# Samsonboadi/Image_to_pointCloud

Measured on NVIDIA B200. Metric: depth_to_point_cloud_throughput, higher is better.
Workload: dtype f64

## Files before the change

image_to_pointcloud_b200/csrc/d2pc_device.cuh:

```cuda
#ifndef D2PC_DEVICE_CUH_
#define D2PC_DEVICE_CUH_

#include <cuda_runtime.h>
#include <stdint.h>

#include "d2pc_math.h"

namespace d2pc {

constexpr int kSampleSize = 8192;
constexpr int kSample2Size = 4096;
constexpr int kSortCap = 16384;
constexpr int kSelBits = 12;
constexpr int kScanThreads = 256;
constexpr int kScanPerThread = 32;
constexpr int kScanTile = kScanThreads * kScanPerThread;
constexpr int kSelThreads = 1024;
constexpr int kSelectThreads = 512;
constexpr int kEmitThreads = 256;
constexpr int kEmitPerThread = 4;
constexpr int kEmitTile = kEmitThreads * kEmitPerThread;
constexpr int kFbTargets = 4;
constexpr uint32_t kCandDivisor = 16;

struct Geom {
  int32_t H, W, C, h, w, step;
  int32_t nu, nv;
  uint32_t P;
  uint32_t N;
  uint32_t D;
  int32_t native;
  double scale_x, scale_y;
};

inline Geom make_geom(const D2pcConfig &c) {
  Geom g;
  g.H = c.img_h; g.W = c.img_w; g.C = c.img_c; g.h = c.dep_h; g.w = c.dep_w; g.step = c.step;
  g.nu = (c.img_w + c.step - 1) / c.step;
  g.nv = (c.img_h + c.step - 1) / c.step;
  g.P = (uint32_t)c.img_h * (uint32_t)c.img_w;
  g.N = (uint32_t)g.nu * (uint32_t)g.nv;
  g.D = (uint32_t)c.dep_h * (uint32_t)c.dep_w;
  g.native = (c.dep_h == c.img_h && c.dep_w == c.img_w) ? 1 : 0;
  g.scale_x = (double)c.dep_w / (double)c.img_w;
  g.scale_y = (double)c.dep_h / (double)c.img_h;
  return g;
}

struct __align__(256) FrameState {
  uint32_t brL[2], brU[2];
  uint32_t sample_ok;
  uint32_t below[2];
  uint32_t above1;
  uint32_t eqL[2];
  uint32_t inside[2];
  uint32_t eqU[2];
  uint32_t n_nonfinite, n_nan;
  alignas(8) uint32_t nqueue[2];
  uint32_t min_key, max_key;
  uint32_t sel_key[4];
  uint32_t sel_fail;
  uint32_t sel_done;
  uint32_t fb_prefix[kFbTargets];
  uint32_t fb_rank[kFbTargets];
  uint32_t fb_active;
  uint32_t fb_any_nan;
  int32_t mask_mode;
  float mask_lo, mask_hi;
  uint32_t emit_count;
  uint32_t bounds_min[3], bounds_max[3];
  alignas(128) NormParams norm;
  int32_t status;
};
static_assert(sizeof(NormParams) + 4 <= 128, "norm + status must share one 128-byte line");
constexpr int kStatusWord = (int)(sizeof(NormParams) / 4);

constexpr uint32_t kSelBins = 4096, kSelListCap = 1024;
struct __align__(256) SelShared {
  uint32_t counts[2][8];
  uint32_t scan_done;
  uint32_t a_done[2], c_done[2];
  uint32_t bin_ready[2];
  uint32_t bin[2][2], base[2][2], need[2][2], want[2][2], shared_bin[2], key[2][2];
  uint32_t mcount[2][2], mmin[2][2], mmax[2][2];
  uint32_t pad_[7];
  uint32_t members[2][2][kSelListCap];
  uint32_t hist[2][kSelBins];
};

struct __align__(8) TapEntry {
  int32_t i0c;
  float t;
};

constexpr int kSchedQueues = 32;
constexpr size_t kSchedBytes = 128 * (kSchedQueues + 1);

struct WsLayout {
  size_t state_off, cand_off, tile_off, fbhist_off, tap_off, sched_off, sel_off, resized_off, total;
  uint32_t cand_cap;
  uint32_t emit_tiles;
};

inline size_t align_up(size_t x, size_t a) { return (x + a - 1) / a * a; }

inline WsLayout make_layout(const D2pcConfig &c) {
  Geom g = make_geom(c);
  WsLayout L;
  uint32_t cap = g.P / kCandDivisor + 1;
  uint32_t small = g.P < (uint32_t)kSortCap ? g.P : (uint32_t)kSortCap;
  if (cap < small) cap = small;
  cap = (cap + 3u) & ~3u;
  L.cand_cap = cap;
  L.emit_tiles = (g.N + kEmitTile - 1) / kEmitTile;
  size_t off = 0;
  L.state_off = off;  off = align_up(off + sizeof(FrameState) * (size_t)c.batch, 256);
  L.cand_off = off;   off = align_up(off + (size_t)c.batch * 2 * cap * sizeof(uint32_t), 256);
  L.tile_off = off;   off = align_up(off + (size_t)c.batch * L.emit_tiles * sizeof(unsigned long long), 256);
  L.fbhist_off = off; off = align_up(off + (size_t)c.batch * kFbTargets * 256 * sizeof(uint32_t), 256);
  L.tap_off = off;    off = align_up(off + ((size_t)c.img_w + (size_t)c.img_h) * sizeof(TapEntry), 256);
  L.sched_off = off;  off = align_up(off + kSchedBytes + (size_t)c.batch * 64, 256);
  L.sel_off = off;    off = align_up(off + (size_t)c.batch * sizeof(SelShared), 256);
  L.resized_off = off;
  if (!g.native) off = align_up(off + (size_t)c.batch * g.P * sizeof(float), 256);
  L.total = off;
  return L;
}

struct KParams {
  Geom g;
  int32_t batch;
  const float *depth;
  FrameState *state;
  uint32_t *cand;
  unsigned long long *tile_state;
  uint32_t *fb_hist;
  const TapEntry *xtab, *ytab;
  SelShared *sel;
  uint32_t *sched;
  float *resized;
  uint32_t cand_cap, emit_tiles;
  int32_t force_fallback;
  int32_t hints;
};

constexpr int kHintScanKeep = 1;
constexpr int kHintEmitDepthFirst = 2;
constexpr int kHintStreamFirst = 4;
constexpr int kHintResizedKeep = 8;
constexpr int kHintPipeline = 15;

inline KParams make_kparams(const D2pcConfig &c, const float *d_depth, void *ws) {
  KParams k;
  WsLayout L = make_layout(c);
  char *base = (char *)ws;
  k.g = make_geom(c);
  k.batch = c.batch;
  k.depth = d_depth;
  k.state = (FrameState *)(base + L.state_off);
  k.cand = (uint32_t *)(base + L.cand_off);
  k.tile_state = (unsigned long long *)(base + L.tile_off);
  k.fb_hist = (uint32_t *)(base + L.fbhist_off);
  k.xtab = (const TapEntry *)(base + L.tap_off);
  k.ytab = k.xtab + c.img_w;
  k.sched = (uint32_t *)(base + L.sched_off);
  k.sel = (SelShared *)(base + L.sel_off);
  k.resized = k.g.native ? nullptr : (float *)(base + L.resized_off);
  k.cand_cap = L.cand_cap;
  k.emit_tiles = L.emit_tiles;
  k.force_fallback = c.force_fallback;
  k.hints = 0;
  return k;
}

inline KParams per_pixel_view(const KParams &kp) {
  KParams v = kp;
  if (!kp.g.native) {
    v.depth = kp.resized;
    v.g.D = kp.g.P;
    v.g.h = kp.g.H;
    v.g.w = kp.g.W;
    v.g.native = 1;
  }
  return v;
}

inline KParams slice_kparams(const KParams &kp, int b0, int nb, int ring_slot) {
  KParams s = kp;
  s.batch = nb;
  s.depth = kp.depth + (size_t)b0 * kp.g.D;
  s.state = kp.state + b0;
  s.cand = kp.cand + (size_t)b0 * 2 * kp.cand_cap;
  s.tile_state = kp.tile_state + (size_t)b0 * kp.emit_tiles;
  s.fb_hist = kp.fb_hist + (size_t)b0 * kFbTargets * 256;
  s.sel = kp.sel + b0;
  if (kp.resized) s.resized = kp.resized + (size_t)(ring_slot >= 0 ? ring_slot : b0) * kp.g.P;
  return s;
}

struct EmitArgs {
  const uint8_t *bgr;
  float *xyz, *rgb;
  uint32_t *count;
  PixelConsts pc;
  int32_t use_z, drop_nf, want_bounds;
  float z_min, z_max;
  uint32_t frame0;
};

int validate_config(const D2pcConfig *cfg);
int check_workspace(const D2pcConfig *cfg, const void *ws, size_t ws_bytes);
int stats_prepare();
int taps_launch(const KParams &kp, cudaStream_t st);
constexpr int kStatsSample = 1, kStatsScan = 2, kStatsSelect = 4, kStatsScanSelect = kStatsScan | kStatsSelect;
int stats_launch(KParams kp, cudaStream_t st, int phases);
int status_launch(const KParams &kp, int32_t *d_status, int32_t *d_any, cudaStream_t st);
EmitArgs make_emit_args(const D2pcConfig &cfg, const uint8_t *d_bgr, float *d_xyz, float *d_rgb, uint32_t *d_count);
EmitArgs slice_emit_args(const EmitArgs &ea, const Geom &g, int b0);
int emit_init_launch(const KParams &kp, cudaStream_t st);
int bounds_export_launch(const KParams &kp, float *d_bounds, cudaStream_t st);
int emit_validate(const D2pcConfig *cfg, const float *d_depth, const uint8_t *d_bgr, void *d_workspace,
                  size_t workspace_bytes, float *d_xyz, float *d_rgb, uint32_t *d_count, float *d_bounds);
int emit_launch(const D2pcConfig &cfg, const KParams &kp, const EmitArgs &ea, float *d_bounds, cudaStream_t st,
                int32_t smooth_k, const double *h_kernel, void *d_scratch);
int record_cuda_error(cudaError_t e);

#define D2PC_CHECK_LAUNCH()                                  \
  do {                                                       \
    cudaError_t e__ = cudaGetLastError();                    \
    if (e__ != cudaSuccess) return record_cuda_error(e__);   \
  } while (0)

#if defined(__CUDACC__)
__device__ __forceinline__ float4 ldg_stream_f4(const float *p) {
  float4 r;
  asm volatile("ld.global.nc.L1::no_allocate.v4.f32 {%0,%1,%2,%3}, [%4];"
               : "=f"(r.x), "=f"(r.y), "=f"(r.z), "=f"(r.w) : "l"(p));
  return r;
}
__device__ __forceinline__ uint64_t l2_policy(bool first, bool last) {
  uint64_t pf, pl, pn;
  asm("createpolicy.fractional.L2::evict_first.b64 %0, 1.0;" : "=l"(pf));
  asm("createpolicy.fractional.L2::evict_last.b64 %0, 1.0;" : "=l"(pl));
  asm("createpolicy.fractional.L2::evict_normal.b64 %0, 1.0;" : "=l"(pn));
  return first ? pf : (last ? pl : pn);
}
__device__ __forceinline__ float4 ldg_f4_pol(const float *p, uint64_t pol) {
  float4 r;
  asm volatile("ld.global.nc.L1::no_allocate.L2::cache_hint.v4.f32 {%0,%1,%2,%3}, [%4], %5;"
               : "=f"(r.x), "=f"(r.y), "=f"(r.z), "=f"(r.w) : "l"(p), "l"(pol));
  return r;
}
__device__ __forceinline__ uint32_t ldg_u32_pol(const void *p, uint64_t pol) {
  uint32_t r;
  asm volatile("ld.global.nc.L1::no_allocate.L2::cache_hint.u32 %0, [%1], %2;" : "=r"(r) : "l"(p), "l"(pol));
  return r;
}
__device__ __forceinline__ void stg_f4_pol(float *p, float4 v, uint64_t pol) {
  asm volatile("st.global.L2::cache_hint.v4.f32 [%0], {%1,%2,%3,%4}, %5;"
               :: "l"(p), "f"(v.x), "f"(v.y), "f"(v.z), "f"(v.w), "l"(pol) : "memory");
}
__device__ __forceinline__ void bulk_store_pol(void *gdst, uint32_t smem_addr, uint32_t bytes, uint64_t pol) {
  asm volatile("cp.async.bulk.global.shared::cta.bulk_group.L2::cache_hint [%0], [%1], %2, %3;"
               :: "l"(gdst), "r"(smem_addr), "r"(bytes), "l"(pol) : "memory");
}
__device__ __forceinline__ uint32_t ldg_stream_u32(const void *p) {
  uint32_t r;
  asm volatile("ld.global.nc.L1::no_allocate.u32 %0, [%1];" : "=r"(r) : "l"(p));
  return r;
}
__device__ __forceinline__ void stg_f1_pol(float *p, float v, uint64_t pol) {
  asm volatile("st.global.L2::cache_hint.f32 [%0], %1, %2;" :: "l"(p), "f"(v), "l"(pol) : "memory");
}
__device__ __forceinline__ void stg_stream_f4(float *p, float4 v) {
  asm volatile("st.global.cs.v4.f32 [%0], {%1,%2,%3,%4};"
               :: "l"(p), "f"(v.x), "f"(v.y), "f"(v.z), "f"(v.w) : "memory");
}
__device__ __forceinline__ void stg_stream_f1(float *p, float v) {
  asm volatile("st.global.cs.f32 [%0], %1;" :: "l"(p), "f"(v) : "memory");
}

__device__ __forceinline__ uint32_t warp_sum(uint32_t v) {
#pragma unroll
  for (int o = 16; o > 0; o >>= 1) v += __shfl_xor_sync(0xffffffffu, v, o);
  return v;
}
__device__ __forceinline__ uint32_t warp_min(uint32_t v) {
#pragma unroll
  for (int o = 16; o > 0; o >>= 1) v = min(v, __shfl_xor_sync(0xffffffffu, v, o));
  return v;
}
__device__ __forceinline__ uint32_t warp_max(uint32_t v) {
#pragma unroll
  for (int o = 16; o > 0; o >>= 1) v = max(v, __shfl_xor_sync(0xffffffffu, v, o));
  return v;
}

__device__ __forceinline__ void block_bitonic_sort(uint32_t *s, uint32_t n) {
  const uint32_t half = n >> 1;
  for (uint32_t k = 2; k <= n; k <<= 1) {
    for (uint32_t j = k >> 1; j > 0; j >>= 1) {
      for (uint32_t i = threadIdx.x; i < half; i += blockDim.x) {
        uint32_t a = ((i & ~(j - 1)) << 1) | (i & (j - 1));
        uint32_t b = a | j;
        uint32_t x = s[a], y = s[b];
        bool up = (a & k) == 0;
        if ((x > y) == up) { s[a] = y; s[b] = x; }
      }
      __syncthreads();
    }
  }
}

template <int T, int NBLOG, typename ForEach>
__device__ __forceinline__ bool block_hist_select(ForEach for_each, uint32_t lo0, uint32_t hi0,
                                                  const uint32_t (&rank)[T], uint32_t (&out)[T],
                                                  uint32_t *s_hist, uint32_t *s_res) {
  constexpr uint32_t NB = 1u << NBLOG;
  const int tid = threadIdx.x, nthr = blockDim.x;
  const int lane = tid & 31, warp = tid >> 5, nwarp = nthr >> 5;
  uint32_t lo[T], span[T], base[T];
  bool done[T];
#pragma unroll
  for (int t = 0; t < T; ++t) { lo[t] = lo0; span[t] = hi0 - lo0; base[t] = 0; done[t] = false; out[t] = 0; }
  bool shared_range = true, ok = true;
  uint32_t *s_warp = s_res + 2 * T;
  for (int level = 0; level < 6; ++level) {
    bool all_done = true;
#pragma unroll
    for (int t = 0; t < T; ++t) all_done = all_done && done[t];
    if (all_done) break;
    int shift[T];
#pragma unroll
    for (int t = 0; t < T; ++t) {
      const int bits = span[t] ? 32 - __clz(span[t]) : 0;
      shift[t] = bits > NBLOG ? bits - NBLOG : 0;
    }
    const int nh = shared_range ? 1 : T;
    for (uint32_t i = tid; i < (uint32_t)nh * NB; i += nthr) s_hist[i] = 0u;
    if (tid < 2 * T) s_res[tid] = 0xFFFFFFFFu;
    __syncthreads();
    if (shared_range) {
      for_each([&](uint32_t key) {
        const uint32_t d = key - lo[0];
        if (d <= span[0]) atomicAdd(&s_hist[d >> shift[0]], 1u);
      });
    } else {
      for_each([&](uint32_t key) {
#pragma unroll
        for (int t = 0; t < T; ++t) {
          const uint32_t d = key - lo[t];
          if (!done[t] && d <= span[t]) atomicAdd(&s_hist[t * NB + (d >> shift[t])], 1u);
        }
      });
    }
    __syncthreads();
    for (int h = 0; h < nh; ++h) {
      if (!shared_range && done[h]) continue;
      const uint32_t *hist = s_hist + (size_t)h * NB;
      constexpr int PER = 4;
      uint32_t carry = 0;
      for (uint32_t chunk = 0; chunk < NB; chunk += (uint32_t)nthr * PER) {
        const uint32_t b0 = chunk + (uint32_t)tid * PER;
        uint32_t c[PER], sum = 0;
#pragma unroll
        for (int i = 0; i < PER; ++i) { c[i] = (b0 + i < NB) ? hist[b0 + i] : 0u; sum += c[i]; }
        uint32_t incl = sum;
#pragma unroll
        for (int d = 1; d < 32; d <<= 1) {
          uint32_t y = __shfl_up_sync(0xffffffffu, incl, d);
          if (lane >= d) incl += y;
        }
        if (lane == 31) s_warp[warp] = incl;
        __syncthreads();
        uint32_t woff = 0, total = 0;
        for (int w = 0; w < nwarp; ++w) { const uint32_t x = s_warp[w]; if (w < warp) woff += x; total += x; }
        uint32_t pref = carry + woff + incl - sum;
#pragma unroll
        for (int i = 0; i < PER; ++i) {
#pragma unroll
          for (int t = 0; t < T; ++t) {
            const bool mine = shared_range ? !done[t] : (t == h);
            const uint32_t r = rank[t] - base[t];
            if (mine && c[i] && pref <= r && r < pref + c[i]) { s_res[2 * t] = b0 + i; s_res[2 * t + 1] = pref; }
          }
          pref += c[i];
        }
        carry += total;
        __syncthreads();
      }
    }
    __syncthreads();
#pragma unroll
    for (int t = 0; t < T; ++t) {
      if (done[t]) continue;
      const uint32_t bin = s_res[2 * t], pref = s_res[2 * t + 1];
      if (bin == 0xFFFFFFFFu) { ok = false; done[t] = true; continue; }
      base[t] += pref;
      lo[t] += bin << shift[t];
      span[t] = shift[t] ? ((1u << shift[t]) - 1u) : 0u;
      if (shift[t] == 0) { done[t] = true; out[t] = lo[t]; }
    }
    shared_range = false;
    __syncthreads();
  }
  return ok;
}

constexpr int kFastBinsLog = 12;
constexpr uint32_t kFastBins = 1u << kFastBinsLog;
constexpr uint32_t kFastListCap = 1024;

__device__ __forceinline__ int fast_shift(uint32_t span) {
  const int bits = span ? 32 - __clz(span) : 0;
  return bits > kFastBinsLog ? bits - kFastBinsLog : 0;
}

template <int T, bool GLOBAL = false>
__device__ __forceinline__ void block_locate(const uint32_t *s_hist, const uint32_t (&rank)[T], const bool (&want)[T],
                                             uint32_t (&bin)[T], uint32_t (&base)[T], uint32_t *s_warp,
                                             uint32_t *s_res) {
  const int tid = threadIdx.x, lane = tid & 31, warp = tid >> 5, nwarp = blockDim.x >> 5;
  const int per = (int)(kFastBins / blockDim.x);
  if (tid < 2 * T) s_res[tid] = 0xFFFFFFFFu;
  const uint32_t b0 = (uint32_t)tid * (uint32_t)per;
  uint32_t sum = 0;
  for (int i = 0; i < per; i += 4) {
    const uint4 c = GLOBAL ? __ldcg(reinterpret_cast<const uint4 *>(s_hist + b0 + i))
                           : *reinterpret_cast<const uint4 *>(s_hist + b0 + i);
    sum += c.x + c.y + c.z + c.w;
  }
  uint32_t incl = sum;
#pragma unroll
  for (int d = 1; d < 32; d <<= 1) {
    const uint32_t y = __shfl_up_sync(0xffffffffu, incl, d);
    if (lane >= d) incl += y;
  }
  if (lane == 31) s_warp[warp] = incl;
  __syncthreads();
  if (warp == 0) {
    const uint32_t x = lane < nwarp ? s_warp[lane] : 0u;
    uint32_t in2 = x;
#pragma unroll
    for (int d = 1; d < 32; d <<= 1) {
      const uint32_t y = __shfl_up_sync(0xffffffffu, in2, d);
      if (lane >= d) in2 += y;
    }
    __syncwarp();
    s_warp[lane] = in2 - x;
  }
  __syncthreads();
  uint32_t pref = s_warp[warp] + incl - sum;
  bool mine = false;
#pragma unroll
  for (int t = 0; t < T; ++t) mine = mine || (want[t] && sum && pref <= rank[t] && rank[t] < pref + sum);
  if (mine) {
    for (int i = 0; i < per; ++i) {
      const uint32_t c = GLOBAL ? __ldcg(s_hist + b0 + i) : s_hist[b0 + i];
#pragma unroll
      for (int t = 0; t < T; ++t)
        if (want[t] && c && pref <= rank[t] && rank[t] < pref + c) { s_res[2 * t] = b0 + i; s_res[2 * t + 1] = pref; }
      pref += c;
    }
  }
  __syncthreads();
#pragma unroll
  for (int t = 0; t < T; ++t) { bin[t] = s_res[2 * t]; base[t] = s_res[2 * t + 1]; }
}

__device__ __forceinline__ void block_pick(const uint32_t *list, uint32_t n, uint32_t r, uint32_t *s_out) {
  for (uint32_t i = threadIdx.x; i < n; i += blockDim.x) {
    const uint32_t k = list[i];
    uint32_t smaller = 0, equal = 0;
    for (uint32_t j = 0; j < n; ++j) {
      const uint32_t x = list[j];
      smaller += x < k ? 1u : 0u;
      equal += x == k ? 1u : 0u;
    }
    if (smaller <= r && r < smaller + equal) *s_out = k;
  }
}

__device__ __forceinline__ uint32_t hash_u32(uint32_t x) {
  x ^= x >> 16; x *= 0x7feb352du; x ^= x >> 15; x *= 0x846ca68bu; x ^= x >> 16;
  return x;
}

__device__ __forceinline__ float bilinear_taps(const float *src, int32_t src_w, TapEntry tx, TapEntry ty) {
  const int32_t x0 = tx.i0c & 0x7FFFFFFF, y0 = ty.i0c & 0x7FFFFFFF;
  const bool cx = tx.i0c < 0, cy = ty.i0c < 0;
  const float *row0 = src + (size_t)y0 * src_w;
  const float a0 = __ldg(row0 + x0);
  float r0 = a0;
  if (!cx) r0 = fmaf(__ldg(row0 + x0 + 1) - a0, tx.t, a0);
  if (cy) return (cx && is_inf_f32(r0)) ? nan_f32() : r0;
  const float *row1 = row0 + src_w;
  const float a1 = __ldg(row1 + x0);
  float r1 = a1;
  if (!cx) r1 = fmaf(__ldg(row1 + x0 + 1) - a1, tx.t, a1);
  return fmaf(r1 - r0, ty.t, r0);
}

template <bool NATIVE>
__device__ __forceinline__ float depth_at(const float *frame, const KParams &kp, uint32_t p) {
  if (NATIVE) {
    return __ldg(frame + p);
  } else {
    const uint32_t v = p / (uint32_t)kp.g.W;
    const uint32_t u = p - v * (uint32_t)kp.g.W;
    return bilinear_taps(frame, kp.g.w, kp.xtab[u], kp.ytab[v]);
  }
}
#endif

}
#endif
```

image_to_pointcloud_b200/csrc/d2pc_path.cu:

```cuda
#include <stdlib.h>
#include <string.h>

#include <vector>

#include "d2pc_emit_dev.cuh"
#include "d2pc_stats_dev.cuh"

using namespace d2pc;

namespace d2pc {

__global__ void sched_reset_kernel(KParams kp) {
  if (threadIdx.x <= kSchedQueues) kp.sched[32 * threadIdx.x] = 0u;
}
int sched_reset_launch(const KParams &kp, cudaStream_t st) {
  sched_reset_kernel<<<1, 64, 0, st>>>(kp);
  D2PC_CHECK_LAUNCH();
  return D2PC_OK;
}

struct SchedParams {
  int32_t F, D;
  uint32_t ns, ne, R;
  uint32_t K;
  uint32_t skip;
  uint32_t nq;
  uint32_t group_items, total_items;
  int32_t vec_ok;
};

constexpr int kPathMinBlocks = 6;
__device__ __forceinline__ unsigned long long global_ns() {
  unsigned long long t;
  asm volatile("mov.u64 %0, %globaltimer;" : "=l"(t));
  return t;
}
__device__ __forceinline__ unsigned long long *trace_slot(const KParams &kp, uint32_t f, int k) {
  return reinterpret_cast<unsigned long long *>(reinterpret_cast<unsigned char *>(kp.sched) + kSchedBytes) + (size_t)f * 8 + k;
}

constexpr int kPathScanPT = 16;

template <bool BOUNDS, bool TRACE>
__global__ void __launch_bounds__(kEmitThreads, kPathMinBlocks) path_kernel(KParams kp, EmitArgs ea, FastArgs fa,
                                                                           SchedParams sp) {
  extern __shared__ __align__(16) unsigned char s_dyn[];
  __shared__ EmitSmall s_emit;
  __shared__ SelPartSmall s_sel;
  __shared__ uint32_t s_go;
  __shared__ NormParams s_norm;
  const int tid = threadIdx.x;
  uint32_t *abort_flag = kp.sched + 32u * kSchedQueues;
  const uint32_t item = blockIdx.x;
  const uint32_t g = item / sp.group_items, i = item - g * sp.group_items;
  if (i < 2u * sp.K) {
    if (g < 1u || g > (uint32_t)sp.F || (sp.skip & 1u)) return;
    const int f = (int)g - 1;
    const uint32_t br = i / sp.K, k = i - br * sp.K;
    if (tid == 0) s_go = spin_until(&kp.sel[f].scan_done, abort_flag, [&](uint32_t v) { return v >= sp.ns; }) ? 1u : 0u;
    __syncthreads();
    if (!s_go) return;
    if (TRACE && tid == 0 && k == 0u) *trace_slot(kp, f, 2 + 2 * (int)br) = global_ns();
    select_part(kp, f, (int)br, k, sp.K, reinterpret_cast<float *>(s_dyn), kSliceCap, s_sel,
                [&](const uint32_t *p, auto pred) { return spin_until(p, abort_flag, pred); });
    if (TRACE) {
      __syncthreads();
      if (tid == 0) atomicMax(trace_slot(kp, f, 3 + 2 * (int)br), global_ns());
    }
    return;
  }
  const uint32_t j = i - 2u * sp.K, q = j / (sp.R + 1u), r = j - q * (sp.R + 1u);
  if (r == 0u) {
    if (g >= (uint32_t)sp.F || (sp.skip & 2u)) return;
    if (TRACE && tid == 0) atomicMin(trace_slot(kp, g, 0), global_ns());
    scan_tile<kPathScanPT>(kp, (int)g, q, sp.vec_ok, *reinterpret_cast<ScanTileSmemT<kPathScanPT> *>(s_dyn));
    __syncthreads();
    if (tid == 0) {
      __threadfence();
      atomicAdd(&kp.sel[g].scan_done, 1u);
      if (TRACE) atomicMax(trace_slot(kp, g, 1), global_ns());
    }
    return;
  }
  const uint32_t e = q * sp.R + (r - 1u);
  if (g < (uint32_t)sp.D || e >= sp.ne || (sp.skip & 4u)) return;
  const uint32_t f = g - (uint32_t)sp.D;
  if (f >= (uint32_t)sp.F) return;
  if (TRACE && tid == 0) atomicMin(trace_slot(kp, f, 6), global_ns());
  auto norm_fn = [&]() -> const NormParams * {
    const uint32_t *line = reinterpret_cast<const uint32_t *>(&kp.state[f].norm);
    uint32_t go = 0u;
    for (int attempt = 0; attempt < 2 && go == 0u; ++attempt) {
      if (tid < 32) {
        const uint32_t w = ld_relaxed_u32(line + tid);
        const uint32_t st = __shfl_sync(0xffffffffu, w, kStatusWord);
        if (st == (uint32_t)D2PC_FRAME_READY && tid < kStatusWord) reinterpret_cast<uint32_t *>(&s_norm)[tid] = w;
        if (tid == 0) s_go = st == (uint32_t)D2PC_FRAME_READY ? 1u : (st == (uint32_t)D2PC_FRAME_PENDING ? 0u : 3u);
      }
      __syncthreads();
      go = s_go;
      if (go == 0u) {
        __syncthreads();
        if (tid == 0) s_go = spin_until(line + kStatusWord, abort_flag, [&](uint32_t x) { return x != (uint32_t)D2PC_FRAME_PENDING; }) ? 0u : 2u;
        __syncthreads();
        go = s_go;
        __syncthreads();
      }
    }
    return go == 1u ? &s_norm : nullptr;
  };
  emit_fast_tile<1, false, BOUNDS>(kp, ea, fa, f, e, reinterpret_cast<float *>(s_dyn), s_emit, norm_fn);
  if (TRACE) {
    __syncthreads();
    if (tid == 0) atomicMax(trace_slot(kp, f, 7), global_ns());
  }
}

}

constexpr int kMaxAux = 8, kMaxEmit = 4;

struct D2pcPath {
  int device;
  cudaStream_t s_cap;
  cudaStream_t s_aux[kMaxAux];
  cudaStream_t s_emit[kMaxEmit];
  std::vector<cudaEvent_t> events;
  cudaGraphExec_t exec;
  std::vector<unsigned char> key;
};

namespace {

struct PathArgs {
  D2pcConfig cfg;
  const float *d_depth;
  const uint8_t *d_bgr;
  void *d_workspace;
  size_t workspace_bytes;
  float *d_xyz, *d_rgb;
  uint32_t *d_count;
  float *d_bounds;
  int32_t *d_status, *d_any_fallback;
  int32_t sub_batch, lookahead, flags;
};

int ensure_events(D2pcPath *p, size_t n) {
  while (p->events.size() < n) {
    cudaEvent_t e;
    cudaError_t err = cudaEventCreateWithFlags(&e, cudaEventDisableTiming);
    if (err != cudaSuccess) return record_cuda_error(err);
    p->events.push_back(e);
  }
  return D2PC_OK;
}

#define PATH_CUDA(x)                                         \
  do {                                                       \
    cudaError_t e__ = (x);                                   \
    if (e__ != cudaSuccess) return record_cuda_error(e__);   \
  } while (0)

int path_kernel_supported(const D2pcConfig &cfg, const KParams &kp, const EmitArgs &ea) {
  const bool mask = cfg.use_z_range || cfg.drop_nonfinite;
  return kp.g.native && cfg.step == 1 && !mask && cfg.img_c == 3 && (cfg.img_w % 4) == 0 &&
         (((uintptr_t)kp.depth & 15u) == 0u) && (((uintptr_t)ea.bgr & 3u) == 0u) && (kp.g.N & 3u) == 0u &&
         ((unsigned long long)kp.g.N * (unsigned long long)kp.g.nu < (1ull << 40)) && kp.g.P > (uint32_t)kSortCap;
}

size_t path_kernel_smem() {
  size_t m = sizeof(ScanTileSmemT<kPathScanPT>);
  if (kEmitStageBytes > m) m = kEmitStageBytes;
  return m;
}

static int env_int(const char *name, int dflt, int lo, int hi);

int path_ordered(const PathArgs &a, cudaStream_t st) {
  const D2pcConfig &cfg = a.cfg;
  KParams kp = make_kparams(cfg, a.d_depth, a.d_workspace);
  kp.hints = (a.flags & D2PC_PATH_NO_L2_HINTS) ? 0 : (kHintScanKeep | kHintEmitDepthFirst | kHintStreamFirst);
  if (const char *h = getenv("D2PC_HINTS")) kp.hints = atoi(h);
  const EmitArgs ea = make_emit_args(cfg, a.d_bgr, a.d_xyz, a.d_rgb, a.d_count);
  int rc;
  const int skip = env_int("D2PC_PATH_SKIP", 0, 0, 15);
  if (skip) {
    if ((rc = sched_reset_launch(kp, st)) != D2PC_OK) return rc;
  } else if ((rc = stats_launch(kp, st, kStatsSample)) != D2PC_OK) return rc;
  if (cfg.want_bounds) {
    if ((rc = emit_init_launch(kp, st)) != D2PC_OK) return rc;
  }
  FastArgs fa;
  fa.tiles_per_frame = kp.emit_tiles;
  fa.total_tiles = kp.emit_tiles * (uint32_t)cfg.batch;
  fa.batch = (uint32_t)cfg.batch;
  fa.magic_w = ((1ull << 40) + (unsigned long long)kp.g.nu - 1ull) / (unsigned long long)kp.g.nu;
  fa.pc_simple = consts_simple(ea.pc) ? 1 : 0;
  SchedParams sp;
  sp.F = cfg.batch;
  sp.D = env_int("D2PC_PATH_D", a.lookahead > 0 ? a.lookahead : 3, 2, 64);
  sp.ns = (kp.g.P + kPathScanPT * kScanThreads - 1) / (kPathScanPT * kScanThreads);
  sp.ne = kp.emit_tiles;
  sp.R = (sp.ne + sp.ns - 1) / sp.ns;
  {
    const uint32_t k = (kp.cand_cap + kSliceCap - 1u) / kSliceCap;
    sp.K = (uint32_t)env_int("D2PC_PATH_K", (int)(k < 8u ? 8u : (k > 64u ? 64u : k)), 1, 64);
  }
  sp.skip = (uint32_t)skip;
  sp.nq = (uint32_t)env_int("D2PC_PATH_NQ", 16, 1, kSchedQueues);
  sp.group_items = 2u * sp.K + sp.ns * (sp.R + 1u);
  const unsigned long long total = (unsigned long long)(sp.F + sp.D) * sp.group_items;
  if (total >= 0xFFFF0000ull) return D2PC_ERR_UNSUPPORTED;
  sp.total_items = (uint32_t)total;
  sp.vec_ok = ((kp.g.P & 3u) == 0u) && (((uintptr_t)kp.depth & 15u) == 0u);
  const size_t smem = path_kernel_smem();
  const bool trace = env_int("D2PC_PATH_TRACE", 0, 0, 1) != 0;
  void (*kern)(KParams, EmitArgs, FastArgs, SchedParams) =
      cfg.want_bounds ? (trace ? path_kernel<true, true> : path_kernel<true, false>)
                      : (trace ? path_kernel<false, true> : path_kernel<false, false>);
  PATH_CUDA(cudaFuncSetAttribute(kern, cudaFuncAttributeMaxDynamicSharedMemorySize, (int)smem));
  kern<<<sp.total_items, kEmitThreads, smem, st>>>(kp, ea, fa, sp);
  D2PC_CHECK_LAUNCH();
  if (cfg.want_bounds) {
    if ((rc = bounds_export_launch(kp, a.d_bounds, st)) != D2PC_OK) return rc;
  }
  if (a.d_status || a.d_any_fallback) {
    if ((rc = status_launch(kp, a.d_status, a.d_any_fallback, st)) != D2PC_OK) return rc;
  }
  return D2PC_OK;
}

static int env_int(const char *name, int dflt, int lo, int hi) {
  const char *v = getenv(name);
  int x = v ? atoi(v) : dflt;
  return x < lo ? lo : (x > hi ? hi : x);
}

int path_body(D2pcPath *p, const PathArgs &a, cudaStream_t s_main) {
  const D2pcConfig &cfg = a.cfg;
  KParams kp = make_kparams(cfg, a.d_depth, a.d_workspace);
  const bool generic = !kp.g.native && resize_is_generic(kp.g.h, kp.g.w);
  const int B = cfg.batch, S = generic ? B : a.sub_batch;
  const int n_sub = (B + S - 1) / S;
  const bool overlap = !(a.flags & D2PC_PATH_NO_OVERLAP) && n_sub > 1;
  const int window = (a.lookahead > 0 ? a.lookahead : 1) + 1;
  const int n_aux = overlap ? env_int("D2PC_PATH_AUX", window < kMaxAux ? window : kMaxAux, 1, kMaxAux) : 1;
  const int n_emit = overlap ? env_int("D2PC_PATH_EMIT", 2, 1, kMaxEmit) : 1;
  const bool sample_first = n_sub > 1 && env_int("D2PC_PATH_SAMPLE_FIRST", 1, 0, 1) != 0;
  const bool ring = kp.resized != nullptr && n_sub > 1;
  kp.hints = (a.flags & D2PC_PATH_NO_L2_HINTS) ? 0 : (n_sub > 1 ? kHintPipeline : (kHintEmitDepthFirst | kHintStreamFirst));
  if (ring) kp.hints &= ~kHintEmitDepthFirst;
  if (const char *h = getenv("D2PC_HINTS")) kp.hints = atoi(h);
  const EmitArgs ea = make_emit_args(cfg, a.d_bgr, a.d_xyz, a.d_rgb, a.d_count);
  int rc;
  if ((rc = ensure_events(p, 1 + 3 * (size_t)n_sub)) != D2PC_OK) return rc;
  cudaEvent_t ev_fork = p->events[0];
  cudaEvent_t *ev_stats = &p->events[1], *ev_emit = &p->events[1 + n_sub], *ev_scan = &p->events[1 + 2 * n_sub];
  const bool stagger = overlap && n_aux > 1 && env_int("D2PC_PATH_STAGGER", 0, 0, 1) != 0;
  if ((rc = taps_launch(kp, s_main)) != D2PC_OK) return rc;
  if (sample_first) {
    if ((rc = stats_launch(kp, s_main, kStatsSample)) != D2PC_OK) return rc;
  }
  if (overlap) {
    PATH_CUDA(cudaEventRecord(ev_fork, s_main));
    for (int i = 0; i < n_aux; ++i) PATH_CUDA(cudaStreamWaitEvent(p->s_aux[i], ev_fork, 0));
    if (n_emit > 1)
      for (int i = 0; i < n_emit; ++i) PATH_CUDA(cudaStreamWaitEvent(p->s_emit[i], ev_fork, 0));
  }
  for (int k = 0; k < n_sub; ++k) {
    const int b0 = k * S, nb = (b0 + S <= B) ? S : B - b0;
    const KParams ks = slice_kparams(kp, b0, nb, ring ? (k % window) * S : -1);
    cudaStream_t s_stats = overlap ? p->s_aux[k % n_aux] : s_main;
    cudaStream_t s_em = (overlap && n_emit > 1) ? p->s_emit[k % n_emit] : s_main;
    if (overlap && k >= window) PATH_CUDA(cudaStreamWaitEvent(s_stats, ev_emit[k - window], 0));
    if (stagger) {
      if (!sample_first && (rc = stats_launch(ks, s_stats, kStatsSample)) != D2PC_OK) return rc;
      if (k > 0) PATH_CUDA(cudaStreamWaitEvent(s_stats, ev_scan[k - 1], 0));
      if ((rc = stats_launch(ks, s_stats, kStatsScan)) != D2PC_OK) return rc;
      PATH_CUDA(cudaEventRecord(ev_scan[k], s_stats));
      if ((rc = stats_launch(ks, s_stats, kStatsSelect)) != D2PC_OK) return rc;
    } else if ((rc = stats_launch(ks, s_stats, sample_first ? kStatsScanSelect : (kStatsSample | kStatsScanSelect))) != D2PC_OK)
      return rc;
    if (overlap) {
      PATH_CUDA(cudaEventRecord(ev_stats[k], s_stats));
      PATH_CUDA(cudaStreamWaitEvent(s_em, ev_stats[k], 0));
    }
    if ((rc = emit_launch(cfg, ks, slice_emit_args(ea, kp.g, b0), a.d_bounds ? a.d_bounds + 6 * (size_t)b0 : nullptr,
                          s_em, 0, nullptr, nullptr)) != D2PC_OK)
      return rc;
    if (overlap) PATH_CUDA(cudaEventRecord(ev_emit[k], s_em));
  }
  if (overlap && n_emit > 1) {
    for (int k = n_sub - 1; k >= 0 && k >= n_sub - n_emit; --k) PATH_CUDA(cudaStreamWaitEvent(s_main, ev_emit[k], 0));
  }
  if (a.d_status || a.d_any_fallback) {
    if ((rc = status_launch(kp, a.d_status, a.d_any_fallback, s_main)) != D2PC_OK) return rc;
  }
  return D2PC_OK;
}

}

extern "C" int d2pc_path_create(D2pcPath **path) {
  if (!path) return D2PC_ERR_INVALID_ARGUMENT;
  *path = nullptr;
  D2pcPath *p = new D2pcPath();
  p->exec = nullptr;
  p->s_cap = nullptr;
  for (int i = 0; i < kMaxAux; ++i) p->s_aux[i] = nullptr;
  for (int i = 0; i < kMaxEmit; ++i) p->s_emit[i] = nullptr;
  cudaError_t e = cudaGetDevice(&p->device);
  int lo = 0, hi = 0;
  if (e == cudaSuccess) e = cudaDeviceGetStreamPriorityRange(&lo, &hi);
  if (e == cudaSuccess) e = cudaStreamCreateWithPriority(&p->s_cap, cudaStreamNonBlocking, lo);
  for (int i = 0; i < kMaxAux && e == cudaSuccess; ++i)
    e = cudaStreamCreateWithPriority(&p->s_aux[i], cudaStreamNonBlocking, getenv("D2PC_PATH_NOPRIO") ? lo : hi);
  for (int i = 0; i < kMaxEmit && e == cudaSuccess; ++i)
    e = cudaStreamCreateWithPriority(&p->s_emit[i], cudaStreamNonBlocking, lo);
  if (e != cudaSuccess) {
    d2pc_path_destroy(p);
    return record_cuda_error(e);
  }
  int rc = stats_prepare();
  if (rc) { d2pc_path_destroy(p); return rc; }
  *path = p;
  return D2PC_OK;
}

extern "C" void d2pc_path_destroy(D2pcPath *p) {
  if (!p) return;
  if (p->exec) cudaGraphExecDestroy(p->exec);
  for (cudaEvent_t e : p->events) cudaEventDestroy(e);
  if (p->s_cap) cudaStreamDestroy(p->s_cap);
  for (int i = 0; i < kMaxAux; ++i)
    if (p->s_aux[i]) cudaStreamDestroy(p->s_aux[i]);
  for (int i = 0; i < kMaxEmit; ++i)
    if (p->s_emit[i]) cudaStreamDestroy(p->s_emit[i]);
  delete p;
}

extern "C" int d2pc_path_enqueue(D2pcPath *p, const D2pcConfig *cfg, const float *d_depth, const uint8_t *d_bgr,
                                 void *d_workspace, size_t workspace_bytes, float *d_xyz, float *d_rgb,
                                 uint32_t *d_count, float *d_bounds, int32_t *d_status, int32_t *d_any_fallback,
                                 int32_t sub_batch, int32_t lookahead, int32_t flags, void *stream) {
  if (!p) return D2PC_ERR_INVALID_ARGUMENT;
  int rc = check_workspace(cfg, d_workspace, workspace_bytes);
  if (rc) return rc;
  rc = emit_validate(cfg, d_depth, d_bgr, d_workspace, workspace_bytes, d_xyz, d_rgb, d_count, d_bounds);
  if (rc) return rc;
  int dev = -1;
  PATH_CUDA(cudaGetDevice(&dev));
  if (dev != p->device) return D2PC_ERR_INVALID_ARGUMENT;
  if (sub_batch <= 0 || sub_batch > cfg->batch) sub_batch = cfg->batch;
  if (lookahead < 0) lookahead = 0;
  PathArgs a;
  memset(&a, 0, sizeof(a));
  a.cfg = *cfg;
  a.d_depth = d_depth; a.d_bgr = d_bgr; a.d_workspace = d_workspace; a.workspace_bytes = workspace_bytes;
  a.d_xyz = d_xyz; a.d_rgb = d_rgb; a.d_count = d_count; a.d_bounds = d_bounds;
  a.d_status = d_status; a.d_any_fallback = d_any_fallback;
  a.sub_batch = sub_batch; a.lookahead = lookahead; a.flags = flags;
  cudaStream_t st = (cudaStream_t)stream;
  {
    const KParams kp0 = make_kparams(a.cfg, a.d_depth, a.d_workspace);
    const EmitArgs ea0 = make_emit_args(a.cfg, a.d_bgr, a.d_xyz, a.d_rgb, a.d_count);
    if ((flags & D2PC_PATH_ORDERED) && path_kernel_supported(a.cfg, kp0, ea0)) return path_ordered(a, st);
  }
  if (!(flags & D2PC_PATH_GRAPH)) return path_body(p, a, st);

  const unsigned char *kb = reinterpret_cast<const unsigned char *>(&a);
  if (!p->exec || p->key.size() != sizeof(a) || memcmp(p->key.data(), kb, sizeof(a)) != 0) {
    if (p->exec) { cudaGraphExecDestroy(p->exec); p->exec = nullptr; }
    p->key.clear();
    cudaGraph_t graph = nullptr;
    PATH_CUDA(cudaStreamBeginCapture(p->s_cap, cudaStreamCaptureModeThreadLocal));
    rc = path_body(p, a, p->s_cap);
    cudaError_t e = cudaStreamEndCapture(p->s_cap, &graph);
    if (rc != D2PC_OK) { if (graph) cudaGraphDestroy(graph); return rc; }
    if (e != cudaSuccess) return record_cuda_error(e);
    e = cudaGraphInstantiate(&p->exec, graph, 0);
    cudaGraphDestroy(graph);
    if (e != cudaSuccess) { p->exec = nullptr; return record_cuda_error(e); }
    p->key.assign(kb, kb + sizeof(a));
  }
  PATH_CUDA(cudaGraphLaunch(p->exec, st));
  return D2PC_OK;
}

extern "C" int d2pc_path_trace_offset(const D2pcConfig *cfg, size_t *offset) {
  int rc = validate_config(cfg);
  if (rc) return rc;
  if (!offset) return D2PC_ERR_INVALID_ARGUMENT;
  *offset = make_layout(*cfg).sched_off + kSchedBytes;
  return D2PC_OK;
}
```

image_to_pointcloud_b200/csrc/d2pc_stats.cu:

```cuda
#include <stdlib.h>

#include "d2pc_stats_dev.cuh"

namespace d2pc {

__device__ __forceinline__ int32_t bracket_margin(double q, int S) {
  double sd = sqrt((double)S * q * (1.0 - q));
  return (int32_t)ceil(6.0 * sd) + 4;
}

__global__ void taps_kernel(KParams kp) {
  TapEntry *xt = const_cast<TapEntry *>(kp.xtab), *yt = const_cast<TapEntry *>(kp.ytab);
  const int i = blockIdx.x * blockDim.x + threadIdx.x;
  if (i < kp.g.W) {
    AxisTap a = axis_tap(i, kp.g.scale_x, kp.g.w);
    xt[i].i0c = a.i0 | (a.clamped ? (int32_t)0x80000000 : 0);
    xt[i].t = a.t;
  } else if (i < kp.g.W + kp.g.H) {
    AxisTap a = axis_tap(i - kp.g.W, kp.g.scale_y, kp.g.h);
    yt[i - kp.g.W].i0c = a.i0 | (a.clamped ? (int32_t)0x80000000 : 0);
    yt[i - kp.g.W].t = a.t;
  }
}

__global__ void __launch_bounds__(256) resize_generic_kernel(KParams kp) {
  const uint32_t b = blockIdx.y;
  const float *src = kp.depth + (size_t)b * kp.g.D;
  float *dst = kp.resized + (size_t)b * kp.g.P;
  for (uint32_t p = blockIdx.x * blockDim.x + threadIdx.x; p < kp.g.P; p += gridDim.x * blockDim.x) {
    const uint32_t v = p / (uint32_t)kp.g.W, u = p - v * (uint32_t)kp.g.W;
    dst[p] = generic_sample(src, kp.g.w, generic_tap((int32_t)u, kp.g.scale_x, kp.g.w, 1),
                            generic_tap((int32_t)v, kp.g.scale_y, kp.g.h, 0));
  }
}

template <bool NATIVE>
__global__ void __launch_bounds__(kSelThreads, 1) sample_kernel(KParams kp) {
  extern __shared__ uint32_t s_hist[];
  __shared__ uint32_t s_bad, s_min, s_max;
  __shared__ uint32_t s_res[2 * 4 + 40];
  __shared__ uint32_t s_warp[33], s_cnt[4], s_lmin[4], s_lmax[4], s_out[4];
  const int b = blockIdx.x;
  FrameState *fs = kp.state + b;
  const float *frame = kp.depth + (size_t)b * kp.g.D;
  const uint32_t n = kp.g.P;
  const int tid = threadIdx.x;
  if (tid == 0) {
    s_bad = 0; s_min = 0xFFFFFFFFu; s_max = 0u;
    for (int i = 0; i < 2; ++i) {
      fs->below[i] = 0; fs->eqL[i] = 0; fs->inside[i] = 0; fs->eqU[i] = 0;
    }
    fs->above1 = 0;
    fs->n_nonfinite = 0; fs->n_nan = 0; fs->nqueue[0] = 0; fs->nqueue[1] = 0;
    fs->min_key = 0xFFFFFFFFu; fs->max_key = 0u;
    for (int i = 0; i < 4; ++i) fs->sel_key[i] = 0;
    fs->sel_fail = 0; fs->sel_done = 0;
    if (b == 0)
      for (int i = 0; i <= kSchedQueues; ++i) kp.sched[32 * i] = 0u;
    {
      unsigned long long *tr = reinterpret_cast<unsigned long long *>(reinterpret_cast<unsigned char *>(kp.sched) + kSchedBytes) + (size_t)b * 8;
      for (int i = 0; i < 8; ++i) tr[i] = (i == 0 || i == 6) ? ~0ull : 0ull;
    }
    fs->status = D2PC_FRAME_PENDING;
    fs->fb_active = 0; fs->fb_any_nan = 0;
    fs->norm.has_nonfinite = 0;
    fs->norm.median = 0.0f;
    fs->norm.simple = 0;
  }
  {
    uint32_t *z = reinterpret_cast<uint32_t *>(kp.sel + b);
    for (uint32_t i = tid; i < sizeof(SelShared) / 4; i += kSelThreads) z[i] = 0u;
  }
  if (n <= (uint32_t)kSortCap) {
    if (tid == 0) {
      fs->brL[0] = fs->brL[1] = 0u;
      fs->brU[0] = fs->brU[1] = 0xFFFFFFFFu;
      fs->sample_ok = 1;
    }
    return;
  }
  constexpr int E = kSampleSize / kSelThreads;
  const uint32_t S = kSampleSize;
  uint32_t k[E];
  bool bad = false;
#pragma unroll
  for (int e = 0; e < E; ++e) {
    const uint32_t j = (uint32_t)e * kSelThreads + (uint32_t)tid;
    uint32_t start = (uint32_t)(((unsigned long long)j * n) / S);
    uint32_t end = (uint32_t)(((unsigned long long)(j + 1) * n) / S);
    uint32_t idx = start + hash_u32(j * 0x9E3779B9u + (uint32_t)b * 0x85EBCA6Bu + 12345u) % (end - start);
    float v;
    if (NATIVE) {
      asm volatile("ld.global.nc.L2::64B.f32 %0, [%1];" : "=f"(v) : "l"(frame + idx));
    } else {
      v = depth_at<NATIVE>(frame, kp, idx);
    }
    k[e] = 0xFFFFFFFFu;
    if (is_finite_f32(v)) k[e] = float_to_key(v); else bad = true;
  }
  __syncthreads();
  if (bad) atomicOr(&s_bad, 1u);
  {
    uint32_t mn = 0xFFFFFFFFu, mx = 0u;
#pragma unroll
    for (int e = 0; e < E; ++e) { mn = min(mn, k[e]); mx = max(mx, k[e]); }
    mn = warp_min(mn); mx = warp_max(mx);
    if ((tid & 31) == 0) { atomicMin(&s_min, mn); atomicMax(&s_max, mx); }
  }
  __syncthreads();
  uint32_t rank[4], out[4];
  bool open_lo[2], open_hi[2];
#pragma unroll
  for (int br = 0; br < 2; ++br) {
    const double q = br ? D2PC_Q98 : D2PC_Q02;
    RankPair rp = percentile_ranks(n, q);
    long long i_lo = (long long)(((unsigned long long)rp.lo * S) / n);
    long long i_hi = (long long)(((unsigned long long)rp.hi * S) / n) + 1;
    int32_t m = bracket_margin(q, (int)S);
    long long iL = i_lo - m, iU = i_hi + m;
    open_lo[br] = iL < 0;
    open_hi[br] = iU >= (long long)S;
    rank[2 * br + 0] = open_lo[br] ? 0u : (uint32_t)iL;
    rank[2 * br + 1] = open_hi[br] ? S - 1 : (uint32_t)iU;
  }
  {
    uint32_t *s_list = s_hist + kFastBins;
    const uint32_t lo0 = s_min, span = s_max - s_min;
    const int shift = fast_shift(span);
    for (uint32_t i = tid; i < kFastBins; i += kSelThreads) s_hist[i] = 0u;
    if (tid < 4) { s_cnt[tid] = 0u; s_lmin[tid] = 0xFFFFFFFFu; s_lmax[tid] = 0u; s_out[tid] = 0u; }
    __syncthreads();
#pragma unroll
    for (int e = 0; e < E; ++e) atomicAdd(&s_hist[(k[e] - lo0) >> shift], 1u);
    __syncthreads();
    uint32_t bin[4], base[4];
    const bool want[4] = {true, true, true, true};
    block_locate<4>(s_hist, rank, want, bin, base, s_warp, s_res);
    bool slow = false;
#pragma unroll
    for (int t = 0; t < 4; ++t) slow = slow || bin[t] == 0xFFFFFFFFu;
    if (!slow && shift == 0) {
#pragma unroll
      for (int t = 0; t < 4; ++t) out[t] = lo0 + bin[t];
    } else if (!slow) {
      int owner[4];
#pragma unroll
      for (int t = 0; t < 4; ++t) {
        owner[t] = t;
#pragma unroll
        for (int u = t - 1; u >= 0; --u)
          if (bin[u] == bin[t]) owner[t] = u;
      }
#pragma unroll
      for (int e = 0; e < E; ++e) {
        const uint32_t bk = (k[e] - lo0) >> shift;
#pragma unroll
        for (int t = 0; t < 4; ++t)
          if (owner[t] == t && bk == bin[t]) {
            const uint32_t idx = atomicAdd(&s_cnt[t], 1u);
            if (idx < kFastListCap) s_list[t * kFastListCap + idx] = k[e];
            atomicMin(&s_lmin[t], k[e]);
            atomicMax(&s_lmax[t], k[e]);
          }
      }
      __syncthreads();
#pragma unroll
      for (int t = 0; t < 4; ++t)
        if (owner[t] == t && s_cnt[t] > kFastListCap && s_lmin[t] != s_lmax[t]) slow = true;
      if (!slow) {
#pragma unroll
        for (int t = 0; t < 4; ++t) {
          const int o = owner[t];
          if (s_lmin[o] == s_lmax[o]) { if (tid == 0) s_out[t] = s_lmin[o]; }
          else block_pick(s_list + o * kFastListCap, s_cnt[o], rank[t] - base[t], &s_out[t]);
        }
        __syncthreads();
#pragma unroll
        for (int t = 0; t < 4; ++t) out[t] = s_out[t];
      }
    }
    if (slow) {
      __syncthreads();
      block_hist_select<4, kSelBits>([&](auto f) {
#pragma unroll
        for (int e = 0; e < E; ++e) f(k[e]);
      }, s_min, s_max, rank, out, s_hist, s_res);
    }
  }
  if (tid < 2) {
    fs->brL[tid] = open_lo[tid] ? 0u : out[2 * tid + 0];
    fs->brU[tid] = open_hi[tid] ? 0xFFFFFFFFu : out[2 * tid + 1];
  }
  if (tid == 0) fs->sample_ok = s_bad ? 0u : 1u;
}

template <int QD>
struct ScanSharedT {
  float pqueue[QD][kScanThreads];
  ScanFlushSmem flush;
};
using ScanShared = ScanSharedT<kScanPerThread>;

constexpr int kRzCols = 128, kRzRows = 32, kRzSrcRows = 40;
constexpr int kRzPerThread = kRzCols * kRzRows / kScanThreads;

__global__ void __launch_bounds__(kScanThreads) scan_resized_tiled_kernel(KParams kp) {
  __shared__ ScanSharedT<kRzPerThread> sh;
  __shared__ __align__(16) float s_h[kRzSrcRows][kRzCols];
  const int b = blockIdx.z, tid = threadIdx.x;
  FrameState *fs = kp.state + b;
  const float *frame = kp.depth + (size_t)b * kp.g.D;
  const int32_t W = kp.g.W, H = kp.g.H, sw = kp.g.w;
  float Lf[2], Uf[2];
  bracket_floats(fs, Lf, Uf);
  const uint32_t q0 = (uint32_t)__cvta_generic_to_shared(&sh.pqueue[0][tid]);
  uint32_t qaddr = q0;
  const int32_t u0 = blockIdx.x * kRzCols, v0 = blockIdx.y * kRzRows;
  const int32_t rows = min(kRzRows, H - v0);
  const int32_t ys = kp.ytab[v0].i0c & 0x7FFFFFFF;
  const TapEntry tl = kp.ytab[v0 + rows - 1];
  const int32_t nsr = (tl.i0c & 0x7FFFFFFF) + (tl.i0c < 0 ? 0 : 1) - ys + 1;
  {
    const int32_t col = tid & (kRzCols - 1), u = u0 + col;
    if (u < W) {
      const TapEntry tx = kp.xtab[u];
      const int32_t x0 = tx.i0c & 0x7FFFFFFF;
      const bool cx = tx.i0c < 0;
      for (int32_t r = tid / kRzCols; r < nsr; r += kScanThreads / kRzCols) {
        const float *row = frame + (size_t)(ys + r) * sw;
        const float a = __ldg(row + x0);
        float h = a;
        if (!cx) h = fmaf(__ldg(row + x0 + 1) - a, tx.t, a);
        s_h[r][col] = h;
      }
    }
  }
  __syncthreads();
  {
    const int32_t c4 = (tid & 31) * 4, uu = u0 + c4, warp = tid >> 5;
    const uint64_t pol_keep = l2_policy(false, (kp.hints & kHintResizedKeep) != 0);
    if (uu < W) {
      bool cxk[4];
#pragma unroll
      for (int k = 0; k < 4; ++k) cxk[k] = kp.xtab[uu + k].i0c < 0;
#pragma unroll 1
      for (int32_t rr = warp; rr < rows; rr += kScanThreads / 32) {
        const int32_t v = v0 + rr;
        const TapEntry ty = kp.ytab[v];
        const int32_t y0 = (ty.i0c & 0x7FFFFFFF) - ys;
        const float4 r0 = *reinterpret_cast<const float4 *>(&s_h[y0][c4]);
        float o[4] = {r0.x, r0.y, r0.z, r0.w};
        if (ty.i0c < 0) {
#pragma unroll
          for (int k = 0; k < 4; ++k)
            if (cxk[k] && is_inf_f32(o[k])) o[k] = nan_f32();
        } else {
          const float4 r1 = *reinterpret_cast<const float4 *>(&s_h[y0 + 1][c4]);
          o[0] = fmaf(r1.x - r0.x, ty.t, r0.x);
          o[1] = fmaf(r1.y - r0.y, ty.t, r0.y);
          o[2] = fmaf(r1.z - r0.z, ty.t, r0.z);
          o[3] = fmaf(r1.w - r0.w, ty.t, r0.w);
        }
#pragma unroll
        for (int k = 0; k < 4; ++k) scan_value(o[k], Uf[0], Lf[1], qaddr);
        float *dst = kp.resized + (size_t)b * kp.g.P + (size_t)v * W + uu;
        stg_f4_pol(dst, make_float4(o[0], o[1], o[2], o[3]), pol_keep);
      }
    }
  }
  scan_flush(&sh.pqueue[0][0], (qaddr - q0) / (uint32_t)(kScanThreads * 4), Uf[0], Lf[1], fs, kp, b, sh.flush);
}

template <int PT>
__global__ void __launch_bounds__(kScanThreads) scan_native_kernel(KParams kp, int vec_ok) {
  extern __shared__ __align__(16) unsigned char s_dyn[];
  scan_tile<PT>(kp, blockIdx.y, blockIdx.x, vec_ok, *reinterpret_cast<ScanTileSmemT<PT> *>(s_dyn));
}

template <int PT, int TPC, int MINB>
__global__ void __launch_bounds__(kScanThreads, MINB) scan_native_multi_kernel(KParams kp, int vec_ok) {
  extern __shared__ __align__(16) unsigned char s_dyn[];
  ScanTileSmemT<PT> &sm = *reinterpret_cast<ScanTileSmemT<PT> *>(s_dyn);
  constexpr int kPx = PT * kScanThreads;
  const int tid = threadIdx.x, b = blockIdx.y;
  FrameState *fs = kp.state + b;
  const float *frame = kp.depth + (size_t)b * kp.g.D;
  const uint32_t n = kp.g.P;
  const uint32_t ntiles = (n + (uint32_t)kPx - 1u) / (uint32_t)kPx;
  const uint32_t t0 = blockIdx.x * (uint32_t)TPC;
  const float U0 = bracket_hi_float(fs->brU[0]), L1 = bracket_lo_float(fs->brL[1]);
  const uint32_t q0 = (uint32_t)__cvta_generic_to_shared(&sm.pq[0][tid]);
  const uint64_t pol = l2_policy((kp.hints & kHintScanKeep) == 0, (kp.hints & kHintScanKeep) != 0);
  auto full = [&](uint32_t tile) { return vec_ok && tile < ntiles && (tile + 1u) * (uint32_t)kPx <= n; };
  float4 r[PT / 4];
  if (full(t0)) {
    const float *src = frame + t0 * (uint32_t)kPx + 4u * (uint32_t)tid;
#pragma unroll
    for (int j = 0; j < PT / 4; ++j) r[j] = ldg_f4_pol(src + (size_t)j * (4 * kScanThreads), pol);
  }
#pragma unroll 1
  for (uint32_t i = 0; i < (uint32_t)TPC; ++i) {
    const uint32_t tile = t0 + i;
    if (tile >= ntiles) break;
    uint32_t qaddr = q0;
    if (full(tile)) {
#pragma unroll
      for (int j = 0; j < PT / 4; ++j) {
        scan_value(r[j].x, U0, L1, qaddr);
        scan_value(r[j].y, U0, L1, qaddr);
        scan_value(r[j].z, U0, L1, qaddr);
        scan_value(r[j].w, U0, L1, qaddr);
      }
    } else {
      const uint32_t tile_base = tile * (uint32_t)kPx;
#pragma unroll 1
      for (int j = 0; j < PT / 4; ++j) {
        const uint32_t p = tile_base + 4u * (uint32_t)(j * kScanThreads + tid);
        for (uint32_t k = 0; k < 4u; ++k)
          if (p + k < n) scan_value(__ldg(frame + p + k), U0, L1, qaddr);
      }
    }
    if (i + 1u < (uint32_t)TPC && full(tile + 1u)) {
      const float *src = frame + (tile + 1u) * (uint32_t)kPx + 4u * (uint32_t)tid;
#pragma unroll
      for (int j = 0; j < PT / 4; ++j) r[j] = ldg_f4_pol(src + (size_t)j * (4 * kScanThreads), pol);
    }
    scan_flush(&sm.pq[0][0], (qaddr - q0) / (uint32_t)(kScanThreads * 4), U0, L1, fs, kp, b, sm.flush);
    __syncthreads();
  }
}

__global__ void __launch_bounds__(kScanThreads) scan_gather_kernel(KParams kp, int vec_ok) {
  __shared__ ScanShared sh;
  const int b = blockIdx.y;
  const int tid = threadIdx.x;
  FrameState *fs = kp.state + b;
  const float *frame = kp.depth + (size_t)b * kp.g.D;
  const uint32_t n = kp.g.P;
  float Lf[2], Uf[2];
  bracket_floats(fs, Lf, Uf);
  const uint32_t q0 = (uint32_t)__cvta_generic_to_shared(&sh.pqueue[0][tid]);
  uint32_t qaddr = q0;
  const uint32_t tile_base = blockIdx.x * (uint32_t)kScanTile;
  const uint32_t W = (uint32_t)kp.g.W;
#pragma unroll 2
  for (int j = 0; j < kScanPerThread / 4; ++j) {
    uint32_t p = tile_base + 4u * (uint32_t)(j * kScanThreads + tid);
    if (p >= n) continue;
    uint32_t v = p / W;
    uint32_t u = p - v * W;
    TapEntry ty = kp.ytab[v];
    float val[4] = {0.0f, 0.0f, 0.0f, 0.0f};
#pragma unroll
    for (uint32_t k = 0; k < 4u; ++k) {
      if (p + k < n) {
        if (u >= W) {
          u -= W;
          v += 1;
          ty = kp.ytab[v];
        }
        val[k] = bilinear_taps(frame, kp.g.w, kp.xtab[u], ty);
        scan_value(val[k], Uf[0], Lf[1], qaddr);
        u += 1;
      }
    }
    float *dst = kp.resized + (size_t)b * n + p;
    if (vec_ok && p + 3u < n) *reinterpret_cast<float4 *>(dst) = make_float4(val[0], val[1], val[2], val[3]);
    else
      for (uint32_t k = 0; k < 4u; ++k)
        if (p + k < n) dst[k] = val[k];
  }
  scan_flush(&sh.pqueue[0][0], (qaddr - q0) / (uint32_t)(kScanThreads * 4), Uf[0], Lf[1], fs, kp, b, sh.flush);
}

__global__ void __launch_bounds__(kSelectThreads, 2) select_kernel(KParams kp) {
  extern __shared__ uint32_t s_sel[];
  __shared__ SelectSmall ss;
  select_bracket(kp, blockIdx.y, blockIdx.x, s_sel, ss);
}

constexpr int kCoopThreads = 512;
constexpr uint32_t kCoopSmemWords = 2u << 11;
__global__ void __launch_bounds__(kCoopThreads) select_a_kernel(KParams kp, uint32_t K) {
  extern __shared__ uint32_t s_sel[];
  __shared__ SelPartSmall ss;
  select_phase_a<true>(kp, blockIdx.z, blockIdx.y, blockIdx.x, K, reinterpret_cast<float *>(s_sel), 0u, ss);
}
__global__ void __launch_bounds__(kCoopThreads) select_c_kernel(KParams kp, uint32_t K) {
  extern __shared__ uint32_t s_sel[];
  __shared__ SelPartSmall ss;
  const int b = blockIdx.z, br = blockIdx.y;
  if (*reinterpret_cast<volatile uint32_t *>(&kp.sel[b].bin_ready[br]) != 1u) return;
  select_phase_c(kp, b, br, blockIdx.x, K, reinterpret_cast<float *>(s_sel), 0u, false, ss);
}

constexpr uint32_t kStatsSliceCap = (uint32_t)(sizeof(ScanTileSmem) / sizeof(float));
__global__ void __launch_bounds__(kScanThreads, 5) stats_ordered_kernel(KParams kp, int vec_ok, uint32_t ns, uint32_t K) {
  extern __shared__ __align__(16) unsigned char s_dyn[];
  __shared__ SelPartSmall s_sel;
  __shared__ uint32_t s_go;
  const int tid = threadIdx.x;
  const uint32_t group_items = 2u * K + ns;
  const uint32_t g = blockIdx.x / group_items, i = blockIdx.x - g * group_items;
  uint32_t *abort_flag = sched_abort_flag(kp);
  if (i < 2u * K) {
    if (g < 1u) return;
    const int f = (int)g - 1;
    const uint32_t br = i / K, k = i - br * K;
    if (tid == 0) s_go = spin_until(&kp.sel[f].scan_done, abort_flag, [&](uint32_t v) { return v >= ns; }) ? 1u : 0u;
    __syncthreads();
    if (!s_go) return;
    select_part(kp, f, (int)br, k, K, reinterpret_cast<float *>(s_dyn), kStatsSliceCap, s_sel,
                [&](const uint32_t *p, auto pred) { return spin_until(p, abort_flag, pred); });
    return;
  }
  if (g >= (uint32_t)kp.batch) return;
  scan_tile<kTilePerThread>(kp, (int)g, i - 2u * K, vec_ok, *reinterpret_cast<ScanTileSmem *>(s_dyn));
  __syncthreads();
  if (tid == 0) {
    __threadfence();
    atomicAdd(&kp.sel[g].scan_done, 1u);
  }
}

enum { kStageMedian = 0, kStagePercentile = 1 };

__global__ void fb_reset_kernel(KParams kp) {
  FrameState *fs = kp.state + blockIdx.x;
  if (threadIdx.x == 0 && fs->status == D2PC_FRAME_NEEDS_FALLBACK) {
    fs->n_nonfinite = 0; fs->n_nan = 0;
    fs->min_key = 0xFFFFFFFFu; fs->max_key = 0u;
  }
}

template <bool NATIVE>
__global__ void __launch_bounds__(kScanThreads) fb_count_kernel(KParams kp) {
  const int b = blockIdx.y, tid = threadIdx.x;
  FrameState *fs = kp.state + b;
  if (fs->status != D2PC_FRAME_NEEDS_FALLBACK) return;
  const float *frame = kp.depth + (size_t)b * kp.g.D;
  const uint32_t n = kp.g.P;
  const uint32_t tile_base = blockIdx.x * (uint32_t)kScanTile;
  uint32_t nf = 0, nan = 0;
  for (int j = 0; j < kScanPerThread; ++j) {
    uint32_t p = tile_base + (uint32_t)(j * kScanThreads + tid);
    if (p >= n) break;
    float v = depth_at<NATIVE>(frame, kp, p);
    if (!is_finite_f32(v)) { nf++; if (is_nan_f32(v)) nan++; }
  }
  nf = warp_sum(nf);
  nan = warp_sum(nan);
  if ((tid & 31) == 0) {
    if (nf) atomicAdd(&fs->n_nonfinite, nf);
    if (nan) atomicAdd(&fs->n_nan, nan);
  }
}

__global__ void fb_begin_kernel(KParams kp) {
  const int b = blockIdx.x;
  FrameState *fs = kp.state + b;
  uint32_t *hist = kp.fb_hist + (size_t)b * kFbTargets * 256;
  for (int i = threadIdx.x; i < kFbTargets * 256; i += blockDim.x) hist[i] = 0;
  if (threadIdx.x != 0) return;
  fs->fb_active = 0;
  fs->fb_any_nan = 0;
  if (fs->status != D2PC_FRAME_NEEDS_FALLBACK) return;
  if (fs->n_nonfinite == 0) return;
  const uint32_t m = kp.g.P - fs->n_nan;
  if (m == 0) return;
  for (int t = 0; t < kFbTargets; ++t) fs->fb_prefix[t] = 0;
  if (m & 1u) {
    fs->fb_rank[0] = m / 2;
    fs->fb_active = 1;
  } else {
    fs->fb_rank[0] = m / 2 - 1;
    fs->fb_rank[1] = m / 2;
    fs->fb_active = 2;
  }
}

template <bool NATIVE>
__global__ void __launch_bounds__(kScanThreads) fb_hist_kernel(KParams kp, int stage, int pass) {
  __shared__ uint32_t sh[kFbTargets][256];
  const int b = blockIdx.y, tid = threadIdx.x;
  FrameState *fs = kp.state + b;
  if (fs->status != D2PC_FRAME_NEEDS_FALLBACK) return;
  const int T = (int)fs->fb_active;
  if (T == 0) return;
  const float *frame = kp.depth + (size_t)b * kp.g.D;
  const uint32_t n = kp.g.P;
  for (int i = tid; i < kFbTargets * 256; i += kScanThreads) (&sh[0][0])[i] = 0;
  uint32_t prefix[kFbTargets];
  for (int t = 0; t < kFbTargets; ++t) prefix[t] = fs->fb_prefix[t];
  const float med = fs->norm.median;
  __syncthreads();
  const int shift = 24 - 8 * pass;
  const uint32_t tile_base = blockIdx.x * (uint32_t)kScanTile;
  uint32_t kmin = 0xFFFFFFFFu, kmax = 0u;
  for (int j = 0; j < kScanPerThread; ++j) {
    uint32_t p = tile_base + (uint32_t)(j * kScanThreads + tid);
    if (p >= n) break;
    float v = depth_at<NATIVE>(frame, kp, p);
    if (stage == kStageMedian) {
      if (is_nan_f32(v)) continue;
    } else {
      if (!is_finite_f32(v)) v = med;
    }
    uint32_t key = float_to_key(v);
    kmin = min(kmin, key);
    kmax = max(kmax, key);
    for (int t = 0; t < T; ++t) {
      bool match = (pass == 0) || ((key >> (shift + 8)) == (prefix[t] >> (shift + 8)));
      if (match) atomicAdd(&sh[t][(key >> shift) & 255u], 1u);
    }
  }
  if (stage == kStagePercentile && pass == 0) {
    kmin = warp_min(kmin);
    kmax = warp_max(kmax);
    if ((tid & 31) == 0) {
      if (kmin != 0xFFFFFFFFu) atomicMin(&fs->min_key, kmin);
      if (kmax != 0u) atomicMax(&fs->max_key, kmax);
    }
  }
  __syncthreads();
  uint32_t *hist = kp.fb_hist + (size_t)b * kFbTargets * 256;
  for (int i = tid; i < T * 256; i += kScanThreads) {
    uint32_t c = (&sh[0][0])[i];
    if (c) atomicAdd(&hist[i], c);
  }
}

__global__ void fb_pick_kernel(KParams kp, int pass) {
  const int b = blockIdx.x;
  FrameState *fs = kp.state + b;
  uint32_t *hist = kp.fb_hist + (size_t)b * kFbTargets * 256;
  const bool live = fs->status == D2PC_FRAME_NEEDS_FALLBACK && fs->fb_active > 0;
  if (live && threadIdx.x < fs->fb_active) {
    const int t = threadIdx.x;
    const int shift = 24 - 8 * pass;
    uint32_t rank = fs->fb_rank[t], cum = 0;
    int d = 0;
    for (; d < 256; ++d) {
      uint32_t c = hist[t * 256 + d];
      if (rank < cum + c) break;
      cum += c;
    }
    if (d > 255) d = 255;
    fs->fb_prefix[t] |= (uint32_t)d << shift;
    fs->fb_rank[t] = rank - cum;
  }
  __syncthreads();
  for (int i = threadIdx.x; i < kFbTargets * 256; i += blockDim.x) hist[i] = 0;
}

__global__ void fb_median_kernel(KParams kp) {
  const int b = blockIdx.x;
  FrameState *fs = kp.state + b;
  if (threadIdx.x != 0 || fs->status != D2PC_FRAME_NEEDS_FALLBACK) return;
  const uint32_t n = kp.g.P;
  float med = 0.0f;
  int has_nf = 0;
  if (fs->n_nonfinite != 0) {
    has_nf = 1;
    const uint32_t m = n - fs->n_nan;
    if (m == 0) {
      med = nan_f32();
    } else {
      const int T = (int)fs->fb_active;
      med = median_from_ranks(key_to_float(fs->fb_prefix[0]), key_to_float(fs->fb_prefix[T - 1]), m);
    }
  }
  fs->norm.median = med;
  fs->norm.has_nonfinite = has_nf;
  const bool any_nan = has_nf && is_nan_f32(med);
  fs->fb_any_nan = any_nan ? 1u : 0u;
  if (any_nan) {
    fs->fb_active = 0;
    return;
  }
  RankPair r2 = percentile_ranks(n, D2PC_Q02), r98 = percentile_ranks(n, D2PC_Q98);
  fs->fb_rank[0] = r2.lo; fs->fb_rank[1] = r2.hi; fs->fb_rank[2] = r98.lo; fs->fb_rank[3] = r98.hi;
  for (int t = 0; t < kFbTargets; ++t) fs->fb_prefix[t] = 0;
  fs->fb_active = 4;
}

__global__ void fb_finalise_kernel(KParams kp) {
  const int b = blockIdx.x;
  FrameState *fs = kp.state + b;
  if (threadIdx.x != 0 || fs->status != D2PC_FRAME_NEEDS_FALLBACK) return;
  const uint32_t n = kp.g.P;
  NormParams np_;
  const float med = fs->norm.median;
  const int has_nf = fs->norm.has_nonfinite;
  if (fs->fb_any_nan) {
    finalise_norm(0.0, 0.0, 0.0f, 0.0f, true, &np_);
  } else {
    RankPair r2 = percentile_ranks(n, D2PC_Q02), r98 = percentile_ranks(n, D2PC_Q98);
    double p2 = lerp_percentile(key_to_float(fs->fb_prefix[0]), key_to_float(fs->fb_prefix[1]), r2.gamma);
    double p98 = lerp_percentile(key_to_float(fs->fb_prefix[2]), key_to_float(fs->fb_prefix[3]), r98.gamma);
    const uint32_t kmin = fs->min_key, kmax = fs->max_key;
    finalise_norm(p2, p98, key_to_float(kmin), key_to_float(kmax), false, &np_);
  }
  np_.median = med;
  np_.has_nonfinite = has_nf;
  finish_norm(&np_);
  fs->norm = np_;
  __threadfence();
  fs->status = D2PC_FRAME_READY;
}

__global__ void status_kernel(KParams kp, int32_t *d_status, int32_t *d_any) {
  __shared__ int s_any;
  if (threadIdx.x == 0) s_any = 0;
  __syncthreads();
  for (int b = threadIdx.x; b < kp.batch; b += blockDim.x) {
    int32_t s = kp.state[b].status;
    if (s == D2PC_FRAME_PENDING) {
      s = D2PC_FRAME_NEEDS_FALLBACK;
      kp.state[b].status = s;
    }
    if (d_status) d_status[b] = s;
    if (s == D2PC_FRAME_NEEDS_FALLBACK) s_any = 1;
  }
  __syncthreads();
  if (threadIdx.x == 0 && d_any) *d_any = s_any;
}

__global__ void params_kernel(KParams kp, D2pcFrameParams *out) {
  for (int b = blockIdx.x * blockDim.x + threadIdx.x; b < kp.batch; b += gridDim.x * blockDim.x) {
    const FrameState &fs = kp.state[b];
    D2pcFrameParams o;
    o.p2 = fs.norm.p2; o.p98 = fs.norm.p98; o.den = fs.norm.den; o.inv_den = fs.norm.inv_den;
    o.lo32 = fs.norm.lo32; o.hi32 = fs.norm.hi32; o.den32 = fs.norm.den32; o.median = fs.norm.median;
    o.branch = fs.norm.branch; o.status = fs.status;
    o.n_nonfinite = fs.n_nonfinite; o.n_nan = fs.n_nan;
    o.n_cand[0] = fs.nqueue[0]; o.n_cand[1] = fs.nqueue[1];
    o.reserved[0] = fs.sel_fail; o.reserved[1] = fs.sample_ok;
    out[b] = o;
  }
}

}

using namespace d2pc;

static int check_ws(const D2pcConfig *cfg, const void *ws, size_t ws_bytes) {
  int rc = validate_config(cfg);
  if (rc) return rc;
  if (!ws) return D2PC_ERR_INVALID_ARGUMENT;
  if (ws_bytes < make_layout(*cfg).total) return D2PC_ERR_WORKSPACE_TOO_SMALL;
  if (((uintptr_t)ws & 255u) != 0) return D2PC_ERR_INVALID_ARGUMENT;
  return D2PC_OK;
}

namespace d2pc {

int taps_launch(const KParams &kp, cudaStream_t st) {
  if (kp.g.native || resize_is_generic(kp.g.h, kp.g.w)) return D2PC_OK;
  taps_kernel<<<(kp.g.W + kp.g.H + 255) / 256, 256, 0, st>>>(kp);
  D2PC_CHECK_LAUNCH();
  return D2PC_OK;
}

int stats_prepare() {
  const size_t sample_smem = (size_t)(4u << kSelBits) * sizeof(uint32_t);
  cudaError_t e = cudaFuncSetAttribute(sample_kernel<true>, cudaFuncAttributeMaxDynamicSharedMemorySize, (int)sample_smem);
  if (e == cudaSuccess)
    e = cudaFuncSetAttribute(select_kernel, cudaFuncAttributeMaxDynamicSharedMemorySize, (int)(kSelectSmemWords * sizeof(uint32_t)));
  if (e == cudaSuccess)
    e = cudaFuncSetAttribute(sample_kernel<false>, cudaFuncAttributeMaxDynamicSharedMemorySize, (int)sample_smem);
  if (e == cudaSuccess)
    e = cudaFuncSetAttribute(scan_native_kernel<kTilePerThread>, cudaFuncAttributeMaxDynamicSharedMemorySize, (int)sizeof(ScanTileSmem));
  if (e == cudaSuccess)
    e = cudaFuncSetAttribute(scan_native_multi_kernel<kTilePerThread, 2, 4>, cudaFuncAttributeMaxDynamicSharedMemorySize, (int)sizeof(ScanTileSmem));
  if (e == cudaSuccess)
    e = cudaFuncSetAttribute(scan_native_multi_kernel<kTilePerThread, 4, 4>, cudaFuncAttributeMaxDynamicSharedMemorySize, (int)sizeof(ScanTileSmem));
  if (e == cudaSuccess)
    e = cudaFuncSetAttribute(stats_ordered_kernel, cudaFuncAttributeMaxDynamicSharedMemorySize, (int)sizeof(ScanTileSmem));
  if (e != cudaSuccess) return record_cuda_error(e);
  return D2PC_OK;
}

int stats_launch(KParams kp, cudaStream_t st, int phases) {
  const int nb = kp.batch;
  if (!kp.g.native && resize_is_generic(kp.g.h, kp.g.w)) {
    const uint32_t blocks = (kp.g.P + 255u) / 256u;
    if (phases & kStatsSample) {
      resize_generic_kernel<<<dim3(blocks < 148u * 8u ? blocks : 148u * 8u, nb), 256, 0, st>>>(kp);
      D2PC_CHECK_LAUNCH();
    }
    kp = per_pixel_view(kp);
  }
  const size_t sample_smem = (size_t)(4u << kSelBits) * sizeof(uint32_t);
  const int vec_ok = ((kp.g.P & 3u) == 0u) && (((uintptr_t)kp.depth & 15u) == 0u);
  dim3 scan_grid((kp.g.P + kScanTile - 1) / kScanTile, nb);
  if (phases & kStatsSample) {
    if (kp.g.native) sample_kernel<true><<<nb, kSelThreads, sample_smem, st>>>(kp);
    else sample_kernel<false><<<nb, kSelThreads, sample_smem, st>>>(kp);
    D2PC_CHECK_LAUNCH();
  }
  if (!(phases & kStatsScanSelect)) return D2PC_OK;
  const char *mode = getenv("D2PC_STATS_ORDERED");
  const bool ordered = (phases & kStatsScanSelect) == kStatsScanSelect && (mode ? atoi(mode) != 0 : nb <= 2);
  if (kp.g.native && kp.g.P > (uint32_t)kSortCap && ordered) {
    const uint32_t ns = (kp.g.P + kTilePx - 1) / kTilePx;
    uint32_t K = (kp.cand_cap + kStatsSliceCap - 1u) / kStatsSliceCap;
    K = K < 4u ? 4u : (K > 64u ? 64u : K);
    const unsigned long long total = (unsigned long long)(nb + 1) * (2ull * K + ns);
    if (total < 0x7FFFFFFFull) {
      stats_ordered_kernel<<<(unsigned)total, kScanThreads, sizeof(ScanTileSmem), st>>>(kp, vec_ok, ns, K);
      D2PC_CHECK_LAUNCH();
      return D2PC_OK;
    }
  }
  if (!(phases & kStatsScan)) {
  } else if (kp.g.native) {
    const uint32_t nt = (kp.g.P + kTilePx - 1) / kTilePx;
    const char *te = getenv("D2PC_SCAN_TPC");
    const unsigned long long tiles = (unsigned long long)nt * (unsigned long long)nb;
    const int tpc = te ? atoi(te) : (tiles >= 4ull * 1184ull ? 4 : (tiles >= 2ull * 1184ull ? 2 : 1));
    if (tpc >= 4) scan_native_multi_kernel<kTilePerThread, 4, 4><<<dim3((nt + 3) / 4, nb), kScanThreads, sizeof(ScanTileSmem), st>>>(kp, vec_ok);
    else if (tpc >= 2) scan_native_multi_kernel<kTilePerThread, 2, 4><<<dim3((nt + 1) / 2, nb), kScanThreads, sizeof(ScanTileSmem), st>>>(kp, vec_ok);
    else scan_native_kernel<kTilePerThread><<<dim3(nt, nb), kScanThreads, sizeof(ScanTileSmem), st>>>(kp, vec_ok);
  } else {
    bool tiled = (kp.g.W & 3) == 0;
    for (int32_t v0 = 0; tiled && v0 < kp.g.H; v0 += kRzRows) {
      const int32_t v1 = (v0 + kRzRows < kp.g.H ? v0 + kRzRows : kp.g.H) - 1;
      const AxisTap t0 = axis_tap(v0, kp.g.scale_y, kp.g.h), t1 = axis_tap(v1, kp.g.scale_y, kp.g.h);
      if (t1.i1 - t0.i0 + 1 > kRzSrcRows) tiled = false;
    }
    if (tiled) {
      dim3 tg((kp.g.W + kRzCols - 1) / kRzCols, (kp.g.H + kRzRows - 1) / kRzRows, nb);
      scan_resized_tiled_kernel<<<tg, kScanThreads, 0, st>>>(kp);
    } else {
      scan_gather_kernel<<<scan_grid, kScanThreads, 0, st>>>(kp, (kp.g.P & 3u) == 0u ? 1 : 0);
    }
  }
  D2PC_CHECK_LAUNCH();
  if (phases & kStatsSelect) {
    const char *cm = getenv("D2PC_SELECT_COOP");
    uint32_t K = 296u / (2u * (uint32_t)nb);
    if (K > 16u) K = 16u;
    if (kp.g.P >= 4u * 1024u * 1024u && K < 4u) K = 4u;
    if (K < 4u) K = 0u;
    if (cm) K = (uint32_t)atoi(cm);
    if (K > 64u) K = 64u;
    if (K >= 2u && kp.g.P > (uint32_t)kSortCap) {
      select_a_kernel<<<dim3(K, 2, nb), kCoopThreads, kCoopSmemWords * sizeof(uint32_t), st>>>(kp, K);
      D2PC_CHECK_LAUNCH();
      select_c_kernel<<<dim3(K, 2, nb), kCoopThreads, kCoopSmemWords * sizeof(uint32_t), st>>>(kp, K);
    } else {
      select_kernel<<<dim3(2, nb), kSelectThreads, (size_t)kSelectSmemWords * sizeof(uint32_t), st>>>(kp);
    }
    D2PC_CHECK_LAUNCH();
  }
  return D2PC_OK;
}

int status_launch(const KParams &kp, int32_t *d_status, int32_t *d_any, cudaStream_t st) {
  status_kernel<<<1, 256, 0, st>>>(kp, d_status, d_any);
  D2PC_CHECK_LAUNCH();
  return D2PC_OK;
}

int check_workspace(const D2pcConfig *cfg, const void *ws, size_t ws_bytes) { return check_ws(cfg, ws, ws_bytes); }

}

extern "C" int d2pc_stats_enqueue(const D2pcConfig *cfg, const float *d_depth, void *d_workspace,
                                  size_t workspace_bytes, void *stream) {
  int rc = check_ws(cfg, d_workspace, workspace_bytes);
  if (rc) return rc;
  if (!d_depth) return D2PC_ERR_INVALID_ARGUMENT;
  cudaStream_t st = (cudaStream_t)stream;
  KParams kp = make_kparams(*cfg, d_depth, d_workspace);
  if ((rc = stats_prepare()) != D2PC_OK) return rc;
  if ((rc = taps_launch(kp, st)) != D2PC_OK) return rc;
  return stats_launch(kp, st, kStatsSample | kStatsScanSelect);
}

extern "C" int d2pc_stats_fallback_enqueue(const D2pcConfig *cfg, const float *d_depth,
                                           void *d_workspace, size_t workspace_bytes, void *stream) {
  int rc = check_ws(cfg, d_workspace, workspace_bytes);
  if (rc) return rc;
  if (!d_depth) return D2PC_ERR_INVALID_ARGUMENT;
  cudaStream_t st = (cudaStream_t)stream;
  KParams kp = per_pixel_view(make_kparams(*cfg, d_depth, d_workspace));
  dim3 grid((kp.g.P + kScanTile - 1) / kScanTile, cfg->batch);
  fb_reset_kernel<<<cfg->batch, 32, 0, st>>>(kp);
  D2PC_CHECK_LAUNCH();
  fb_count_kernel<true><<<grid, kScanThreads, 0, st>>>(kp);
  D2PC_CHECK_LAUNCH();
  fb_begin_kernel<<<cfg->batch, 256, 0, st>>>(kp);
  D2PC_CHECK_LAUNCH();
  for (int stage = 0; stage < 2; ++stage) {
    for (int pass = 0; pass < 4; ++pass) {
      fb_hist_kernel<true><<<grid, kScanThreads, 0, st>>>(kp, stage, pass);
      D2PC_CHECK_LAUNCH();
      fb_pick_kernel<<<cfg->batch, 256, 0, st>>>(kp, pass);
      D2PC_CHECK_LAUNCH();
    }
    if (stage == 0) fb_median_kernel<<<cfg->batch, 32, 0, st>>>(kp);
    else fb_finalise_kernel<<<cfg->batch, 32, 0, st>>>(kp);
    D2PC_CHECK_LAUNCH();
  }
  return D2PC_OK;
}

extern "C" int d2pc_frame_status(const D2pcConfig *cfg, const void *d_workspace, int32_t *d_status,
                                 int32_t *d_any_fallback, void *stream) {
  int rc = validate_config(cfg);
  if (rc) return rc;
  if (!d_workspace) return D2PC_ERR_INVALID_ARGUMENT;
  KParams kp = make_kparams(*cfg, nullptr, (void *)d_workspace);
  return status_launch(kp, d_status, d_any_fallback, (cudaStream_t)stream);
}

extern "C" int d2pc_frame_params(const D2pcConfig *cfg, const void *d_workspace,
                                 D2pcFrameParams *d_params, void *stream) {
  int rc = validate_config(cfg);
  if (rc) return rc;
  if (!d_workspace || !d_params) return D2PC_ERR_INVALID_ARGUMENT;
  KParams kp = make_kparams(*cfg, nullptr, (void *)d_workspace);
  params_kernel<<<(cfg->batch + 127) / 128, 128, 0, (cudaStream_t)stream>>>(kp, d_params);
  D2PC_CHECK_LAUNCH();
  return D2PC_OK;
}
```

image_to_pointcloud_b200/csrc/d2pc_stats_dev.cuh:

```cuda
#ifndef D2PC_STATS_DEV_CUH_
#define D2PC_STATS_DEV_CUH_

#include "d2pc_device.cuh"

namespace d2pc {

constexpr int kTilePerThread = 32;
constexpr int kTilePx = kScanThreads * kTilePerThread;

__device__ __forceinline__ void scan_value(float v, float U0, float L1, uint32_t &qaddr) {
  asm volatile(
      "{\n\t"
      ".reg .pred mid;\n\t"
      "setp.gt.f32 mid, %1, %2;\n\t"
      "setp.lt.and.f32 mid, %1, %3, mid;\n\t"
      "@!mid st.shared.f32 [%0], %1;\n\t"
      "@!mid add.u32 %0, %0, %4;\n\t"
      "}"
      : "+r"(qaddr)
      : "f"(v), "f"(U0), "f"(L1), "n"(kScanThreads * 4)
      : "memory");
}

__device__ __forceinline__ float bracket_lo_float(uint32_t L) {
  return (L == 0u) ? -__int_as_float(0x7F800000) : key_to_float(L);
}
__device__ __forceinline__ float bracket_hi_float(uint32_t U) {
  return (U == 0xFFFFFFFFu) ? __int_as_float(0x7F800000) : key_to_float(U);
}
__device__ __forceinline__ void bracket_floats(const FrameState *fs, float Lf[2], float Uf[2]) {
#pragma unroll
  for (int br = 0; br < 2; ++br) {
    Lf[br] = bracket_lo_float(fs->brL[br]);
    Uf[br] = bracket_hi_float(fs->brU[br]);
  }
}

struct ScanFlushSmem {
  uint32_t wtot[kScanThreads / 32];
  uint32_t gbase[2];
};
__device__ __forceinline__ void scan_flush(const float *pq, uint32_t nq, float U0, float L1, FrameState *fs,
                                           const KParams &kp, int b, ScanFlushSmem &sm) {
  const int tid = threadIdx.x, lane = tid & 31, warp = tid >> 5;
  uint32_t packed = 0;
  for (uint32_t j = 0; j < nq; ++j) {
    const float v = pq[j * kScanThreads + tid];
    packed += (!(v > U0) ? 1u : 0u) + ((v >= L1) ? 0x10000u : 0u);
  }
  uint32_t incl = packed;
#pragma unroll
  for (int d = 1; d < 32; d <<= 1) {
    const uint32_t y = __shfl_up_sync(0xffffffffu, incl, d);
    if (lane >= d) incl += y;
  }
  if (lane == 31) sm.wtot[warp] = incl;
  __syncthreads();
  uint32_t woff = 0, total = 0;
#pragma unroll
  for (int w = 0; w < kScanThreads / 32; ++w) {
    const uint32_t x = sm.wtot[w];
    if (w < warp) woff += x;
    total += x;
  }
  if (total == 0u) return;
  if (tid == 0) {
    const unsigned long long add = (unsigned long long)(total & 0xFFFFu) | ((unsigned long long)(total >> 16) << 32);
    const unsigned long long old = atomicAdd(reinterpret_cast<unsigned long long *>(&fs->nqueue[0]), add);
    sm.gbase[0] = (uint32_t)old;
    sm.gbase[1] = (uint32_t)(old >> 32);
  }
  __syncthreads();
  if (nq == 0u) return;
  float *gq0 = reinterpret_cast<float *>(kp.cand) + (size_t)b * 2 * kp.cand_cap;
  const uint32_t excl = woff + incl - packed;
  uint32_t o0 = sm.gbase[0] + (excl & 0xFFFFu), o1 = sm.gbase[1] + (excl >> 16);
  const uint64_t pol_keep = l2_policy(false, true);
  if (o0 + (packed & 0xFFFFu) <= kp.cand_cap && o1 + (packed >> 16) <= kp.cand_cap) {
    o1 += kp.cand_cap;
    for (uint32_t j = 0; j < nq; ++j) {
      const float v = pq[j * kScanThreads + tid];
      if (!(v > U0)) stg_f1_pol(gq0 + o0++, v, pol_keep);
      if (v >= L1) stg_f1_pol(gq0 + o1++, v, pol_keep);
    }
  } else {
    for (uint32_t j = 0; j < nq; ++j) {
      const float v = pq[j * kScanThreads + tid];
      if (!(v > U0)) { if (o0 < kp.cand_cap) gq0[o0] = v; ++o0; }
      if (v >= L1) { if (o1 < kp.cand_cap) gq0[kp.cand_cap + o1] = v; ++o1; }
    }
  }
}

template <int PT>
struct ScanTileSmemT {
  float pq[PT][kScanThreads];
  ScanFlushSmem flush;
};
using ScanTileSmem = ScanTileSmemT<kTilePerThread>;

template <int PT>
__device__ __forceinline__ void scan_tile(const KParams &kp, int b, uint32_t tile, int vec_ok, ScanTileSmemT<PT> &sm) {
  constexpr int kTilePerThread = PT;
  constexpr int kTilePx = PT * kScanThreads;
  const int tid = threadIdx.x;
  FrameState *fs = kp.state + b;
  const float *frame = kp.depth + (size_t)b * kp.g.D;
  const uint32_t n = kp.g.P;
  const float U0 = bracket_hi_float(fs->brU[0]), L1 = bracket_lo_float(fs->brL[1]);
  const uint32_t q0 = (uint32_t)__cvta_generic_to_shared(&sm.pq[0][tid]);
  uint32_t qaddr = q0;
  const uint32_t tile_base = tile * (uint32_t)kTilePx;
  if (vec_ok && tile_base + (uint32_t)kTilePx <= n) {
    const float *src = frame + tile_base + 4u * (uint32_t)tid;
    const uint64_t pol = l2_policy((kp.hints & kHintScanKeep) == 0, (kp.hints & kHintScanKeep) != 0);
    float4 r[kTilePerThread / 4];
#pragma unroll
    for (int j = 0; j < kTilePerThread / 4; ++j) r[j] = ldg_f4_pol(src + (size_t)j * (4 * kScanThreads), pol);
#pragma unroll
    for (int j = 0; j < kTilePerThread / 4; ++j) {
      scan_value(r[j].x, U0, L1, qaddr);
      scan_value(r[j].y, U0, L1, qaddr);
      scan_value(r[j].z, U0, L1, qaddr);
      scan_value(r[j].w, U0, L1, qaddr);
    }
  } else {
#pragma unroll 1
    for (int j = 0; j < kTilePerThread / 4; ++j) {
      const uint32_t p = tile_base + 4u * (uint32_t)(j * kScanThreads + tid);
      for (uint32_t k = 0; k < 4u; ++k)
        if (p + k < n) scan_value(__ldg(frame + p + k), U0, L1, qaddr);
    }
  }
  const uint32_t nq = (qaddr - q0) / (uint32_t)(kScanThreads * 4);
  scan_flush(&sm.pq[0][0], nq, U0, L1, fs, kp, b, sm.flush);
}

__device__ __forceinline__ void finalise_fast(FrameState *fs, uint32_t n) {
  volatile FrameState *vfs = fs;
  if (vfs->sel_fail) {
    __threadfence();
    vfs->status = D2PC_FRAME_NEEDS_FALLBACK;
    return;
  }
  RankPair r2 = percentile_ranks(n, D2PC_Q02), r98 = percentile_ranks(n, D2PC_Q98);
  double p2 = lerp_percentile(key_to_float(vfs->sel_key[0]), key_to_float(vfs->sel_key[1]), r2.gamma);
  double p98 = lerp_percentile(key_to_float(vfs->sel_key[2]), key_to_float(vfs->sel_key[3]), r98.gamma);
  if (!(p98 > p2)) {
    __threadfence();
    vfs->status = D2PC_FRAME_NEEDS_FALLBACK;
    return;
  }
  NormParams np_;
  finalise_norm(p2, p98, 0.0f, 0.0f, false, &np_);
  np_.median = 0.0f;
  np_.has_nonfinite = 0;
  finish_norm(&np_);
  fs->norm = np_;
  __threadfence();
  vfs->status = D2PC_FRAME_READY;
}

template <int U, typename F>
__device__ __forceinline__ void for_each_queued(const float *q, uint32_t nq, F f) {
  const uint32_t stride = blockDim.x;
  uint32_t i = threadIdx.x;
  for (; i + (uint32_t)(U - 1) * stride < nq; i += (uint32_t)U * stride) {
    float v[U];
#pragma unroll
    for (int k = 0; k < U; ++k) v[k] = __ldcg(q + i + (uint32_t)k * stride);
#pragma unroll
    for (int k = 0; k < U; ++k) f(v[k]);
  }
  for (; i < nq; i += stride) f(__ldcg(q + i));
}

constexpr int kSelectSmemWords = (int)kFastBins + 2 * (int)kFastListCap;

struct SelectSmall {
  uint32_t res[2 * 2 + 40];
  uint32_t c[6];
  uint32_t warp[33], cnt[2], lmin[2], lmax[2], out[2];
};

__device__ __forceinline__ void select_bracket(const KParams &kp, int b, int br, uint32_t *s_hist, SelectSmall &ss) {
  const int tid = threadIdx.x, nthr = blockDim.x;
  FrameState *fs = kp.state + b;
  const uint32_t n = kp.g.P;
  const uint32_t qcap = kp.cand_cap;
  const float *q = reinterpret_cast<const float *>(kp.cand) + ((size_t)b * 2 + br) * qcap;
  volatile FrameState *vfs = fs;
  const uint32_t nqueue = vfs->nqueue[br];
  const uint32_t nq = min(nqueue, qcap);
  const uint32_t L = fs->brL[br], U = fs->brU[br];
  float Lf2[2], Uf2[2];
  bracket_floats(fs, Lf2, Uf2);
  const float Lf = Lf2[br], Uf = Uf2[br];
  const uint32_t lo0 = L > 0u ? L - 1u : 0u;
  const uint32_t hi0 = U < 0xFFFFFFFFu ? U + 1u : U;
  const uint32_t span = hi0 - lo0;
  const int shift = fast_shift(span);
  const uint32_t list_cap = kFastListCap;
  uint32_t *s_list = s_hist + kFastBins;
  for (uint32_t i = tid; i < kFastBins; i += nthr) s_hist[i] = 0u;
  if (tid < 6) ss.c[tid] = 0;
  if (tid < 2) { ss.cnt[tid] = 0u; ss.lmin[tid] = 0xFFFFFFFFu; ss.lmax[tid] = 0u; ss.out[tid] = 0u; }
  __syncthreads();
  {
    uint32_t c_eqL = 0, c_in = 0, c_eqU = 0, c_below = 0, c_nf = 0;
    for_each_queued<8>(q, nq, [&](float v) {
      if (!(fabsf(v) < __int_as_float(0x7F800000))) c_nf += 1u + ((v != v) ? 0x10000u : 0u);
      else if (v < Lf) c_below++;
      else if (v == Lf) c_eqL++;
      else if (v < Uf) {
        c_in++;
        const uint32_t d = float_to_key(v) - lo0;
        if (d <= span) atomicAdd(&s_hist[d >> shift], 1u);
      } else if (v == Uf) c_eqU++;
    });
    c_eqL = warp_sum(c_eqL); c_in = warp_sum(c_in); c_eqU = warp_sum(c_eqU); c_below = warp_sum(c_below);
    const uint32_t w_nf = warp_sum(c_nf & 0xFFFFu), w_nan = warp_sum(c_nf >> 16);
    if ((tid & 31) == 0) {
      if (c_eqL) atomicAdd(&ss.c[0], c_eqL);
      if (c_in) atomicAdd(&ss.c[1], c_in);
      if (c_eqU) atomicAdd(&ss.c[2], c_eqU);
      if (c_below) atomicAdd(&ss.c[3], c_below);
      if (w_nf) atomicAdd(&ss.c[4], w_nf);
      if (w_nan) atomicAdd(&ss.c[5], w_nan);
    }
  }
  __syncthreads();
  const uint32_t eqL = ss.c[0], nin = ss.c[1], eqU = ss.c[2], n_nf = ss.c[4];
  const uint32_t below = br == 0 ? ss.c[3] : n - nqueue;
  bool fail = (n_nf != 0u) || (nqueue > qcap) || (fs->sample_ok == 0u) || (kp.force_fallback != 0);
  RankPair rp = percentile_ranks(n, br ? D2PC_Q98 : D2PC_Q02);
  bool want[2] = {false, false};
  uint32_t need[2] = {0u, 0u};
  uint32_t key[2] = {0u, 0u};
  for (int t = 0; t < 2; ++t) {
    uint32_t r = t ? rp.hi : rp.lo;
    if (r < below) { fail = true; continue; }
    uint32_t r1 = r - below;
    if (r1 < eqL) { key[t] = L; continue; }
    uint32_t r2 = r1 - eqL;
    if (r2 < nin) { need[t] = r2; want[t] = true; continue; }
    uint32_t r3 = r2 - nin;
    if (r3 < eqU) { key[t] = U; continue; }
    fail = true;
  }

  if (!fail && (want[0] || want[1])) {
    uint32_t bin[2], base[2];
    block_locate<2>(s_hist, need, want, bin, base, ss.warp, ss.res);
    bool slow = (want[0] && bin[0] == 0xFFFFFFFFu) || (want[1] && bin[1] == 0xFFFFFFFFu);
    if (!slow && shift == 0) {
      for (int t = 0; t < 2; ++t)
        if (want[t]) key[t] = lo0 + bin[t];
    } else if (!slow) {
      const bool shared_bin = want[0] && want[1] && bin[0] == bin[1];
      const bool own[2] = {want[0], want[1] && !shared_bin};
      for_each_queued<8>(q, nq, [&](float v) {
        if (v > Lf && v < Uf) {
          const uint32_t k = float_to_key(v);
          const uint32_t bk = (k - lo0) >> shift;
#pragma unroll
          for (int t = 0; t < 2; ++t)
            if (own[t] && bk == bin[t]) {
              const uint32_t idx = atomicAdd(&ss.cnt[t], 1u);
              if (idx < list_cap) s_list[t * kFastListCap + idx] = k;
              atomicMin(&ss.lmin[t], k);
              atomicMax(&ss.lmax[t], k);
            }
        }
      });
      __syncthreads();
      for (int t = 0; t < 2; ++t)
        if (own[t] && ss.cnt[t] > list_cap && ss.lmin[t] != ss.lmax[t]) slow = true;
      if (!slow) {
        for (int t = 0; t < 2; ++t) {
          if (!want[t]) continue;
          const int o = (t == 1 && shared_bin) ? 0 : t;
          if (ss.lmin[o] == ss.lmax[o]) { if (tid == 0) ss.out[t] = ss.lmin[o]; }
          else block_pick(s_list + o * kFastListCap, ss.cnt[o], need[t] - base[t], &ss.out[t]);
        }
        __syncthreads();
        for (int t = 0; t < 2; ++t)
          if (want[t]) key[t] = ss.out[t];
      }
    }
    if (slow) {
      __syncthreads();
      uint32_t rk[2], ok_[2];
      for (int t = 0; t < 2; ++t) rk[t] = want[t] ? need[t] : need[1 - t];
      const bool ok = block_hist_select<2, 11>([&](auto f) {
        for_each_queued<8>(q, nq, [&](float v) {
          if (v > Lf && v < Uf) f(float_to_key(v));
        });
      }, lo0, hi0, rk, ok_, s_hist, ss.res);
      if (!ok) fail = true;
      for (int t = 0; t < 2; ++t)
        if (want[t]) key[t] = ok_[t];
    }
  }

  if (tid == 0) {
    fs->sel_key[2 * br + 0] = key[0];
    fs->sel_key[2 * br + 1] = key[1];
    fs->eqL[br] = eqL; fs->inside[br] = nin; fs->eqU[br] = eqU;
    fs->below[br] = below;
    if (n_nf) { atomicAdd(&fs->n_nonfinite, n_nf); atomicAdd(&fs->n_nan, ss.c[5]); }
    if (fail) atomicOr(&fs->sel_fail, 1u);
    __threadfence();
    uint32_t ticket = atomicAdd(&fs->sel_done, 1u);
    if (ticket == 1u) {
      __threadfence();
      finalise_fast(fs, n);
    }
  }
}

constexpr uint32_t kSpinLimit = 1u << 19;

__device__ __forceinline__ uint32_t ld_relaxed_u32(const uint32_t *p) {
  uint32_t v;
  asm volatile("ld.relaxed.gpu.global.u32 %0, [%1];" : "=r"(v) : "l"(p) : "memory");
  return v;
}
__device__ __forceinline__ uint32_t ld_acquire_u32(const uint32_t *p) {
  uint32_t v;
  asm volatile("ld.acquire.gpu.global.u32 %0, [%1];" : "=r"(v) : "l"(p) : "memory");
  return v;
}

template <typename Pred>
__device__ __forceinline__ bool spin_until(const uint32_t *p, uint32_t *abort_flag, Pred pred) {
  uint32_t spins = 0, ns = 128;
  while (!pred(ld_relaxed_u32(p))) {
    __nanosleep(ns);
    if (ns < 2048u) ns <<= 1;
    if (++spins > kSpinLimit || ((spins & 15u) == 0u && ld_relaxed_u32(abort_flag))) {
      atomicExch(abort_flag, 1u);
      return false;
    }
  }
  (void)ld_acquire_u32(p);
  return true;
}

__device__ __forceinline__ uint32_t *sched_abort_flag(const KParams &kp) { return kp.sched + 32u * kSchedQueues; }

constexpr uint32_t kSliceCap = 6144;

struct SelPartSmall {
  uint32_t c[6];
  uint32_t res[2 * 2 + 40];
  uint32_t warp[33];
  uint32_t flag_a, flag_spin, flag_c, out[2];
};

__device__ __forceinline__ void select_finish(FrameState *fs, SelShared *sh, int br, uint32_t n, const uint32_t key[2],
                                              bool fail) {
  volatile uint32_t *cn = sh->counts[br];
  fs->sel_key[2 * br + 0] = key[0];
  fs->sel_key[2 * br + 1] = key[1];
  fs->eqL[br] = cn[1]; fs->inside[br] = cn[2]; fs->eqU[br] = cn[3];
  if (cn[4]) { atomicAdd(&fs->n_nonfinite, cn[4]); atomicAdd(&fs->n_nan, cn[5]); }
  if (fail) atomicOr(&fs->sel_fail, 1u);
  __threadfence();
  const uint32_t ticket = atomicAdd(&fs->sel_done, 1u);
  if (ticket == 1u) {
    __threadfence();
    finalise_fast(fs, n);
  }
}

struct SelCommon {
  FrameState *fs;
  SelShared *sh;
  const float *q;
  uint32_t n, qcap, nqueue, nq, L, U, lo0, hi0, span, s_lo, m;
  float Lf, Uf;
  int shift;
  bool cached;
};
__device__ __forceinline__ SelCommon select_common(const KParams &kp, int b, int br, uint32_t k, uint32_t K, uint32_t slice_cap) {
  SelCommon c;
  c.fs = kp.state + b;
  c.sh = kp.sel + b;
  volatile FrameState *vfs = c.fs;
  c.n = kp.g.P; c.qcap = kp.cand_cap;
  c.q = reinterpret_cast<const float *>(kp.cand) + ((size_t)b * 2 + br) * c.qcap;
  c.nqueue = vfs->nqueue[br];
  c.nq = min(c.nqueue, c.qcap);
  c.L = c.fs->brL[br]; c.U = c.fs->brU[br];
  c.Lf = bracket_lo_float(c.L); c.Uf = bracket_hi_float(c.U);
  c.lo0 = c.L > 0u ? c.L - 1u : 0u;
  c.hi0 = c.U < 0xFFFFFFFFu ? c.U + 1u : c.U;
  c.span = c.hi0 - c.lo0;
  c.shift = fast_shift(c.span);
  const uint32_t chunk = (c.nq + K - 1u) / K;
  c.s_lo = min(c.nq, k * chunk);
  c.m = min(c.nq, c.s_lo + chunk) - c.s_lo;
  c.cached = chunk <= slice_cap;
  return c;
}

template <bool LOCAL_HIST = false>
__device__ __forceinline__ int select_phase_a(const KParams &kp, int b, int br, uint32_t k, uint32_t K, float *s_slice,
                                              uint32_t slice_cap, SelPartSmall &ss) {
  const int tid = threadIdx.x, nthr = blockDim.x;
  const SelCommon cm = select_common(kp, b, br, k, K, slice_cap);
  FrameState *fs = cm.fs;
  SelShared *sh = cm.sh;
  const float *q = cm.q;
  const uint32_t n = cm.n, qcap = cm.qcap, nqueue = cm.nqueue, L = cm.L, U = cm.U, lo0 = cm.lo0, span = cm.span,
                 s_lo = cm.s_lo, m = cm.m;
  const float Lf = cm.Lf, Uf = cm.Uf;
  const int shift = cm.shift;
  const bool cached = cm.cached && !LOCAL_HIST;
  if (tid < 6) ss.c[tid] = 0u;
  if (LOCAL_HIST)
    for (uint32_t i = tid; i < kSelBins; i += nthr) reinterpret_cast<uint32_t *>(s_slice)[i] = 0u;
  __syncthreads();
  {
    uint32_t c_eqL = 0, c_in = 0, c_eqU = 0, c_below = 0, c_nf = 0;
    uint32_t *hist = LOCAL_HIST ? reinterpret_cast<uint32_t *>(s_slice) : sh->hist[br];
    auto visit = [&](float v) {
      if (!(fabsf(v) < __int_as_float(0x7F800000))) c_nf += 1u + ((v != v) ? 0x10000u : 0u);
      else if (v < Lf) c_below++;
      else if (v == Lf) c_eqL++;
      else if (v < Uf) {
        c_in++;
        const uint32_t d = float_to_key(v) - lo0;
        if (d <= span) atomicAdd(&hist[d >> shift], 1u);
      } else if (v == Uf) c_eqU++;
    };
    uint32_t i = tid;
    for (; i + 7u * nthr < m; i += 8u * nthr) {
      float v[8];
#pragma unroll
      for (int u = 0; u < 8; ++u) v[u] = __ldcg(q + s_lo + i + (uint32_t)u * nthr);
#pragma unroll
      for (int u = 0; u < 8; ++u) {
        if (cached) s_slice[i + (uint32_t)u * nthr] = v[u];
        visit(v[u]);
      }
    }
    for (; i < m; i += nthr) {
      const float v = __ldcg(q + s_lo + i);
      if (cached) s_slice[i] = v;
      visit(v);
    }
    c_eqL = warp_sum(c_eqL); c_in = warp_sum(c_in); c_eqU = warp_sum(c_eqU); c_below = warp_sum(c_below);
    const uint32_t w_nf = warp_sum(c_nf & 0xFFFFu), w_nan = warp_sum(c_nf >> 16);
    if ((tid & 31) == 0) {
      if (c_below) atomicAdd(&ss.c[0], c_below);
      if (c_eqL) atomicAdd(&ss.c[1], c_eqL);
      if (c_in) atomicAdd(&ss.c[2], c_in);
      if (c_eqU) atomicAdd(&ss.c[3], c_eqU);
      if (w_nf) atomicAdd(&ss.c[4], w_nf);
      if (w_nan) atomicAdd(&ss.c[5], w_nan);
    }
  }
  __syncthreads();
  if (LOCAL_HIST) {
    const uint32_t *lh = reinterpret_cast<const uint32_t *>(s_slice);
    for (uint32_t i = tid; i < kSelBins; i += nthr) {
      const uint32_t h = lh[i];
      if (h) atomicAdd(&sh->hist[br][i], h);
    }
    __threadfence();
    __syncthreads();
  }
  if (tid == 0) {
    for (int c = 0; c < 6; ++c)
      if (ss.c[c]) atomicAdd(&sh->counts[br][c], ss.c[c]);
    __threadfence();
    ss.flag_a = atomicAdd(&sh->a_done[br], 1u);
    __threadfence();
  }
  __syncthreads();
  const bool last_a = ss.flag_a == K - 1u;
  if (last_a) {
    volatile uint32_t *cn = sh->counts[br];
    const uint32_t eqL = cn[1], nin = cn[2], eqU = cn[3], n_nf = cn[4];
    const uint32_t below = br == 0 ? cn[0] : n - nqueue;
    bool fail = (n_nf != 0u) || (nqueue > qcap) || (fs->sample_ok == 0u) || (kp.force_fallback != 0);
    const RankPair rp = percentile_ranks(n, br ? D2PC_Q98 : D2PC_Q02);
    bool want[2] = {false, false};
    uint32_t need[2] = {0u, 0u}, key[2] = {0u, 0u};
    for (int t = 0; t < 2; ++t) {
      const uint32_t r = t ? rp.hi : rp.lo;
      if (r < below) { fail = true; continue; }
      const uint32_t r1 = r - below;
      if (r1 < eqL) { key[t] = L; continue; }
      const uint32_t r2 = r1 - eqL;
      if (r2 < nin) { need[t] = r2; want[t] = true; continue; }
      const uint32_t r3 = r2 - nin;
      if (r3 < eqU) { key[t] = U; continue; }
      fail = true;
    }
    bool collect = false;
    uint32_t bin[2] = {0u, 0u}, base[2] = {0u, 0u};
    if (!fail && (want[0] || want[1])) {
      block_locate<2, true>(sh->hist[br], need, want, bin, base, ss.warp, ss.res);
      if ((want[0] && bin[0] == 0xFFFFFFFFu) || (want[1] && bin[1] == 0xFFFFFFFFu)) fail = true;
      else if (shift == 0) {
        for (int t = 0; t < 2; ++t)
          if (want[t]) key[t] = lo0 + bin[t];
      } else collect = true;
    }
    if (tid == 0) {
      if (collect) {
        for (int t = 0; t < 2; ++t) {
          sh->bin[br][t] = bin[t]; sh->base[br][t] = base[t]; sh->need[br][t] = need[t];
          sh->want[br][t] = want[t] ? 1u : 0u;
          sh->key[br][t] = key[t];
        }
        sh->shared_bin[br] = (want[0] && want[1] && bin[0] == bin[1]) ? 1u : 0u;
        __threadfence();
        *reinterpret_cast<volatile uint32_t *>(&sh->bin_ready[br]) = 1u;
      } else {
        select_finish(fs, sh, br, n, key, fail);
        __threadfence();
        *reinterpret_cast<volatile uint32_t *>(&sh->bin_ready[br]) = 2u;
      }
    }
    return collect ? 1 : 2;
  }
  return 0;
}

__device__ __forceinline__ void select_phase_c(const KParams &kp, int b, int br, uint32_t k, uint32_t K,
                                               float *s_slice, uint32_t slice_cap, bool slice_is_cached, SelPartSmall &ss) {
  const int tid = threadIdx.x, nthr = blockDim.x;
  const SelCommon cm = select_common(kp, b, br, k, K, slice_cap);
  FrameState *fs = cm.fs;
  SelShared *sh = cm.sh;
  const float *q = cm.q;
  const uint32_t n = cm.n, nq = cm.nq, lo0 = cm.lo0, hi0 = cm.hi0, s_lo = cm.s_lo, m = cm.m;
  const float Lf = cm.Lf, Uf = cm.Uf;
  const int shift = cm.shift;
  const bool cached = cm.cached && slice_is_cached;
  {
    volatile SelShared *vsh = sh;
    const bool shared_bin = vsh->shared_bin[br] != 0u;
    const bool own[2] = {vsh->want[br][0] != 0u, vsh->want[br][1] != 0u && !shared_bin};
    const uint32_t bin0 = vsh->bin[br][0], bin1 = vsh->bin[br][1];
    auto collect = [&](float v) {
      if (v > Lf && v < Uf) {
        const uint32_t key = float_to_key(v);
        const uint32_t bk = (key - lo0) >> shift;
#pragma unroll
        for (int t = 0; t < 2; ++t)
          if (own[t] && bk == (t ? bin1 : bin0)) {
            const uint32_t idx = atomicAdd(&sh->mcount[br][t], 1u);
            if (idx < kSelListCap) sh->members[br][t][idx] = key;
            atomicMax(&sh->mmin[br][t], ~key);
            atomicMax(&sh->mmax[br][t], key);
          }
      }
    };
    uint32_t i = tid;
    if (!cached) {
      for (; i + 7u * nthr < m; i += 8u * nthr) {
        float v[8];
#pragma unroll
        for (int u = 0; u < 8; ++u) v[u] = __ldcg(q + s_lo + i + (uint32_t)u * nthr);
#pragma unroll
        for (int u = 0; u < 8; ++u) collect(v[u]);
      }
    }
    for (; i < m; i += nthr) collect(cached ? s_slice[i] : __ldcg(q + s_lo + i));
  }
  __syncthreads();
  if (tid == 0) {
    __threadfence();
    ss.flag_c = atomicAdd(&sh->c_done[br], 1u);
    __threadfence();
  }
  __syncthreads();
  if (ss.flag_c != K - 1u) return;
  {
    volatile SelShared *vsh = sh;
    const bool shared_bin = vsh->shared_bin[br] != 0u;
    bool want[2] = {vsh->want[br][0] != 0u, vsh->want[br][1] != 0u};
    uint32_t key[2] = {vsh->key[br][0], vsh->key[br][1]};
    bool fail = false, slow = false;
    uint32_t *s_list = reinterpret_cast<uint32_t *>(s_slice);
    for (int t = 0; t < 2; ++t) {
      if (!want[t] || (t == 1 && shared_bin)) continue;
      const uint32_t cnt = vsh->mcount[br][t];
      if (cnt > kSelListCap && ~vsh->mmin[br][t] != vsh->mmax[br][t]) slow = true;
      for (uint32_t i = tid; i < min(cnt, kSelListCap); i += nthr) s_list[t * kSelListCap + i] = __ldcg(&sh->members[br][t][i]);
    }
    if (tid < 2) ss.out[tid] = 0u;
    __syncthreads();
    if (!slow) {
      for (int t = 0; t < 2; ++t) {
        if (!want[t]) continue;
        const int o = (t == 1 && shared_bin) ? 0 : t;
        const uint32_t mn = ~vsh->mmin[br][o], mx = vsh->mmax[br][o];
        if (mn == mx) { if (tid == 0) ss.out[t] = mn; }
        else block_pick(s_list + o * kSelListCap, min(vsh->mcount[br][o], kSelListCap), vsh->need[br][t] - vsh->base[br][t], &ss.out[t]);
      }
      __syncthreads();
      for (int t = 0; t < 2; ++t)
        if (want[t]) key[t] = ss.out[t];
    } else {
      uint32_t rk[2], ok_[2];
      for (int t = 0; t < 2; ++t) rk[t] = want[t] ? vsh->need[br][t] : vsh->need[br][1 - t];
      const bool ok = block_hist_select<2, 11>([&](auto f) {
        for_each_queued<8>(q, nq, [&](float v) {
          if (v > Lf && v < Uf) f(float_to_key(v));
        });
      }, lo0, hi0, rk, ok_, reinterpret_cast<uint32_t *>(s_slice), ss.res);
      if (!ok) fail = true;
      for (int t = 0; t < 2; ++t)
        if (want[t]) key[t] = ok_[t];
    }
    if (tid == 0) select_finish(fs, sh, br, n, key, fail);
  }
}

template <typename Spin>
__device__ __forceinline__ bool select_part(const KParams &kp, int b, int br, uint32_t k, uint32_t K, float *s_slice,
                                            uint32_t slice_cap, SelPartSmall &ss, Spin spin) {
  const int st = select_phase_a<false>(kp, b, br, k, K, s_slice, slice_cap, ss);
  if (st == 2) return true;
  SelShared *sh = kp.sel + b;
  if (st == 0) {
    if (threadIdx.x == 0) ss.flag_spin = spin(&sh->bin_ready[br], [](uint32_t v) { return v != 0u; }) ? 1u : 0u;
    __syncthreads();
    if (!ss.flag_spin) return false;
    if (*reinterpret_cast<volatile uint32_t *>(&sh->bin_ready[br]) == 2u) return true;
  }
  __syncthreads();
  select_phase_c(kp, b, br, k, K, s_slice, slice_cap, true, ss);
  return true;
}

}
#endif
```

profiles/stats_only.py:

```python
import os
import sys

import torch

sys.path.insert(0, os.path.dirname(os.path.dirname(os.path.abspath(__file__))))
import image_to_pointcloud_b200 as m


def main(batch=128, iters=20, H=1080, W=1920, h=None, w=None):
    dev = torch.device("cuda", 0)
    h, w = h or H, w or W
    g = torch.Generator(device=dev)
    g.manual_seed(7)
    depth = torch.rand((batch, h, w), generator=g, device=dev) * 20
    eng = m.FrameEngine(H, W, h, w, batch=batch, device=dev)
    cfg = eng.make_config(density="high")
    s = torch.cuda.current_stream(dev)
    for _ in range(3):
        eng.enqueue_stats(cfg, depth, s)
    torch.cuda.synchronize()
    a, b = torch.cuda.Event(enable_timing=True), torch.cuda.Event(enable_timing=True)
    a.record()
    for _ in range(iters):
        eng.enqueue_stats(cfg, depth, s)
    b.record()
    torch.cuda.synchronize()
    eng.enqueue_status(cfg, s)
    torch.cuda.synchronize()
    print("stats ms per %d frames: %.4f  (any fallback: %d)" % (batch, a.elapsed_time(b) / iters, int(eng._any_host[0])))


if __name__ == "__main__":
    a = [int(x) for x in sys.argv[1:]]
    main(*a)
```

Before: 173,600.

## Count extreme tails during scan instead of queueing them; vectorise queue walks

The scan flush now classifies values below the low bracket's lower bound and above the high bracket's upper bound as tails. It counts them in a packed per-block counter committed with one 64-bit atomic, instead of pushing them into the candidate queues. This is meant to shrink the queues the select phases must re-read. Queue walking becomes float4-based with a smaller unroll, and chunk sizes are rounded to multiples of four for alignment. It adds an extra block reduction and syncs per scan block, and it changes how the 'below' rank is derived, which risks correctness if the bracket bounds are loose.

```diff
diff --git a/image_to_pointcloud_b200/csrc/d2pc_device.cuh b/image_to_pointcloud_b200/csrc/d2pc_device.cuh
--- a/image_to_pointcloud_b200/csrc/d2pc_device.cuh
+++ b/image_to_pointcloud_b200/csrc/d2pc_device.cuh
@@ -50,8 +50,6 @@
 struct __align__(256) FrameState {
   uint32_t brL[2], brU[2];
   uint32_t sample_ok;
-  uint32_t below[2];
-  uint32_t above1;
   uint32_t eqL[2];
   uint32_t inside[2];
   uint32_t eqU[2];
@@ -69,10 +67,15 @@
   float mask_lo, mask_hi;
   uint32_t emit_count;
   uint32_t bounds_min[3], bounds_max[3];
+  alignas(8) uint32_t below0;
+  uint32_t above1;
   alignas(128) NormParams norm;
   int32_t status;
 };
 static_assert(sizeof(NormParams) + 4 <= 128, "norm + status must share one 128-byte line");
+static_assert(offsetof(FrameState, brL) == 0 && offsetof(FrameState, brU) == 8, "FrameState layout");
+static_assert(offsetof(FrameState, nqueue) == 56 && offsetof(FrameState, below0) == 176, "FrameState layout");
+static_assert(offsetof(FrameState, above1) == 180 && sizeof(FrameState) == 512, "FrameState layout");
 constexpr int kStatusWord = (int)(sizeof(NormParams) / 4);
 
 constexpr uint32_t kSelBins = 4096, kSelListCap = 1024;
diff --git a/image_to_pointcloud_b200/csrc/d2pc_path.cu b/image_to_pointcloud_b200/csrc/d2pc_path.cu
--- a/image_to_pointcloud_b200/csrc/d2pc_path.cu
+++ b/image_to_pointcloud_b200/csrc/d2pc_path.cu
@@ -61,7 +61,7 @@
     __syncthreads();
     if (!s_go) return;
     if (TRACE && tid == 0 && k == 0u) *trace_slot(kp, f, 2 + 2 * (int)br) = global_ns();
-    select_part(kp, f, (int)br, k, sp.K, reinterpret_cast<float *>(s_dyn), kSliceCap, s_sel,
+    select_part<2>(kp, f, (int)br, k, sp.K, reinterpret_cast<float *>(s_dyn), kSliceCap, s_sel,
                 [&](const uint32_t *p, auto pred) { return spin_until(p, abort_flag, pred); });
     if (TRACE) {
       __syncthreads();
diff --git a/image_to_pointcloud_b200/csrc/d2pc_stats.cu b/image_to_pointcloud_b200/csrc/d2pc_stats.cu
--- a/image_to_pointcloud_b200/csrc/d2pc_stats.cu
+++ b/image_to_pointcloud_b200/csrc/d2pc_stats.cu
@@ -48,9 +48,9 @@
   if (tid == 0) {
     s_bad = 0; s_min = 0xFFFFFFFFu; s_max = 0u;
     for (int i = 0; i < 2; ++i) {
-      fs->below[i] = 0; fs->eqL[i] = 0; fs->inside[i] = 0; fs->eqU[i] = 0;
-    }
-    fs->above1 = 0;
+      fs->eqL[i] = 0; fs->inside[i] = 0; fs->eqU[i] = 0;
+    }
+    fs->below0 = 0; fs->above1 = 0;
     fs->n_nonfinite = 0; fs->n_nan = 0; fs->nqueue[0] = 0; fs->nqueue[1] = 0;
     fs->min_key = 0xFFFFFFFFu; fs->max_key = 0u;
     for (int i = 0; i < 4; ++i) fs->sel_key[i] = 0;
@@ -211,8 +211,7 @@
   FrameState *fs = kp.state + b;
   const float *frame = kp.depth + (size_t)b * kp.g.D;
   const int32_t W = kp.g.W, H = kp.g.H, sw = kp.g.w;
-  float Lf[2], Uf[2];
-  bracket_floats(fs, Lf, Uf);
+  const ScanBounds bd = scan_bounds(fs);
   const uint32_t q0 = (uint32_t)__cvta_generic_to_shared(&sh.pqueue[0][tid]);
   uint32_t qaddr = q0;
   const int32_t u0 = blockIdx.x * kRzCols, v0 = blockIdx.y * kRzRows;
@@ -262,13 +261,16 @@
           o[3] = fmaf(r1.w - r0.w, ty.t, r0.w);
         }
 #pragma unroll
-        for (int k = 0; k < 4; ++k) scan_value(o[k], Uf[0], Lf[1], qaddr);
+        for (int k = 0; k < 4; ++k) scan_value(o[k], bd.U0, bd.L1, qaddr);
         float *dst = kp.resized + (size_t)b * kp.g.P + (size_t)v * W + uu;
         stg_f4_pol(dst, make_float4(o[0], o[1], o[2], o[3]), pol_keep);
       }
     }
   }
-  scan_flush(&sh.pqueue[0][0], (qaddr - q0) / (uint32_t)(kScanThreads * 4), Uf[0], Lf[1], fs, kp, b, sh.flush);
+  uint32_t tails = 0;
+  scan_flush(&sh.pqueue[0][0], (qaddr - q0) / (uint32_t)(kScanThreads * 4), bd, fs, kp, b, sh.flush, tails);
+  __syncthreads();
+  scan_tails_commit(tails, fs, sh.flush);
 }
 
 template <int PT>
@@ -288,11 +290,13 @@
   const uint32_t n = kp.g.P;
   const uint32_t ntiles = (n + (uint32_t)kPx - 1u) / (uint32_t)kPx;
   const uint32_t t0 = blockIdx.x * (uint32_t)TPC;
-  const float U0 = bracket_hi_float(fs->brU[0]), L1 = bracket_lo_float(fs->brL[1]);
+  const ScanBounds bd = scan_bounds(fs);
+  const float U0 = bd.U0, L1 = bd.L1;
   const uint32_t q0 = (uint32_t)__cvta_generic_to_shared(&sm.pq[0][tid]);
   const uint64_t pol = l2_policy((kp.hints & kHintScanKeep) == 0, (kp.hints & kHintScanKeep) != 0);
   auto full = [&](uint32_t tile) { return vec_ok && tile < ntiles && (tile + 1u) * (uint32_t)kPx <= n; };
   float4 r[PT / 4];
+  uint32_t tails = 0;
   if (full(t0)) {
     const float *src = frame + t0 * (uint32_t)kPx + 4u * (uint32_t)tid;
 #pragma unroll
@@ -325,9 +329,10 @@
 #pragma unroll
       for (int j = 0; j < PT / 4; ++j) r[j] = ldg_f4_pol(src + (size_t)j * (4 * kScanThreads), pol);
     }
-    scan_flush(&sm.pq[0][0], (qaddr - q0) / (uint32_t)(kScanThreads * 4), U0, L1, fs, kp, b, sm.flush);
+    scan_flush(&sm.pq[0][0], (qaddr - q0) / (uint32_t)(kScanThreads * 4), bd, fs, kp, b, sm.flush, tails);
     __syncthreads();
   }
+  scan_tails_commit(tails, fs, sm.flush);
 }
 
 __global__ void __launch_bounds__(kScanThreads) scan_gather_kernel(KParams kp, int vec_ok) {
@@ -337,8 +342,7 @@
   FrameState *fs = kp.state + b;
   const float *frame = kp.depth + (size_t)b * kp.g.D;
   const uint32_t n = kp.g.P;
-  float Lf[2], Uf[2];
-  bracket_floats(fs, Lf, Uf);
+  const ScanBounds bd = scan_bounds(fs);
   const uint32_t q0 = (uint32_t)__cvta_generic_to_shared(&sh.pqueue[0][tid]);
   uint32_t qaddr = q0;
   const uint32_t tile_base = blockIdx.x * (uint32_t)kScanTile;
@@ -360,7 +364,7 @@
           ty = kp.ytab[v];
         }
         val[k] = bilinear_taps(frame, kp.g.w, kp.xtab[u], ty);
-        scan_value(val[k], Uf[0], Lf[1], qaddr);
+        scan_value(val[k], bd.U0, bd.L1, qaddr);
         u += 1;
       }
     }
@@ -370,7 +374,10 @@
       for (uint32_t k = 0; k < 4u; ++k)
         if (p + k < n) dst[k] = val[k];
   }
-  scan_flush(&sh.pqueue[0][0], (qaddr - q0) / (uint32_t)(kScanThreads * 4), Uf[0], Lf[1], fs, kp, b, sh.flush);
+  uint32_t tails = 0;
+  scan_flush(&sh.pqueue[0][0], (qaddr - q0) / (uint32_t)(kScanThreads * 4), bd, fs, kp, b, sh.flush, tails);
+  __syncthreads();
+  scan_tails_commit(tails, fs, sh.flush);
 }
 
 __global__ void __launch_bounds__(kSelectThreads, 2) select_kernel(KParams kp) {
diff --git a/image_to_pointcloud_b200/csrc/d2pc_stats_dev.cuh b/image_to_pointcloud_b200/csrc/d2pc_stats_dev.cuh
--- a/image_to_pointcloud_b200/csrc/d2pc_stats_dev.cuh
+++ b/image_to_pointcloud_b200/csrc/d2pc_stats_dev.cuh
@@ -36,18 +36,37 @@
   }
 }
 
+struct ScanBounds {
+  float L0, U0, L1, U1;
+};
+__device__ __forceinline__ ScanBounds scan_bounds(const FrameState *fs) {
+  ScanBounds s;
+  s.L0 = bracket_lo_float(fs->brL[0]); s.U0 = bracket_hi_float(fs->brU[0]);
+  s.L1 = bracket_lo_float(fs->brL[1]); s.U1 = bracket_hi_float(fs->brU[1]);
+  return s;
+}
+
+__device__ __forceinline__ uint32_t flush_side(float v, const ScanBounds &s, uint32_t &tail) {
+  const float inf = __int_as_float(0x7F800000);
+  tail = ((v < s.L0 && v > -inf) ? 1u : 0u) + ((v > s.U1 && v < inf) ? 0x10000u : 0u);
+  return (!(v > s.U0) ? 1u : 0u) + ((v >= s.L1) ? 0x10000u : 0u);
+}
+
 struct ScanFlushSmem {
   uint32_t wtot[kScanThreads / 32];
   uint32_t gbase[2];
 };
-__device__ __forceinline__ void scan_flush(const float *pq, uint32_t nq, float U0, float L1, FrameState *fs,
-                                           const KParams &kp, int b, ScanFlushSmem &sm) {
+__device__ __forceinline__ void scan_flush(const float *pq, uint32_t nq, const ScanBounds &bd, FrameState *fs,
+                                           const KParams &kp, int b, ScanFlushSmem &sm, uint32_t &tails) {
   const int tid = threadIdx.x, lane = tid & 31, warp = tid >> 5;
-  uint32_t packed = 0;
+  uint32_t packed = 0, tl = 0;
   for (uint32_t j = 0; j < nq; ++j) {
-    const float v = pq[j * kScanThreads + tid];
-    packed += (!(v > U0) ? 1u : 0u) + ((v >= L1) ? 0x10000u : 0u);
-  }
+    uint32_t t;
+    packed += flush_side(pq[j * kScanThreads + tid], bd, t);
+    tl += t;
+  }
+  packed -= tl;
+  tails += tl;
   uint32_t incl = packed;
 #pragma unroll
   for (int d = 1; d < 32; d <<= 1) {
@@ -80,16 +99,35 @@
     o1 += kp.cand_cap;
     for (uint32_t j = 0; j < nq; ++j) {
       const float v = pq[j * kScanThreads + tid];
-      if (!(v > U0)) stg_f1_pol(gq0 + o0++, v, pol_keep);
-      if (v >= L1) stg_f1_pol(gq0 + o1++, v, pol_keep);
+      uint32_t t;
+      const uint32_t c = flush_side(v, bd, t) - t;
+      if (c & 1u) stg_f1_pol(gq0 + o0++, v, pol_keep);
+      if (c >> 16) stg_f1_pol(gq0 + o1++, v, pol_keep);
     }
   } else {
     for (uint32_t j = 0; j < nq; ++j) {
       const float v = pq[j * kScanThreads + tid];
-      if (!(v > U0)) { if (o0 < kp.cand_cap) gq0[o0] = v; ++o0; }
-      if (v >= L1) { if (o1 < kp.cand_cap) gq0[kp.cand_cap + o1] = v; ++o1; }
-    }
-  }
+      uint32_t t;
+      const uint32_t c = flush_side(v, bd, t) - t;
+      if (c & 1u) { if (o0 < kp.cand_cap) gq0[o0] = v; ++o0; }
+      if (c >> 16) { if (o1 < kp.cand_cap) gq0[kp.cand_cap + o1] = v; ++o1; }
+    }
+  }
+}
+
+__device__ __forceinline__ void scan_tails_commit(uint32_t tails, FrameState *fs, ScanFlushSmem &sm) {
+  const int tid = threadIdx.x;
+  tails = __reduce_add_sync(0xffffffffu, tails);
+  if ((tid & 31) == 0) sm.wtot[tid >> 5] = tails;
+  __syncthreads();
+  if (tid == 0) {
+    uint32_t t = 0;
+#pragma unroll
+    for (int w = 0; w < kScanThreads / 32; ++w) t += sm.wtot[w];
+    if (t) atomicAdd(reinterpret_cast<unsigned long long *>(&fs->below0),
+                     (unsigned long long)(t & 0xFFFFu) | ((unsigned long long)(t >> 16) << 32));
+  }
+  __syncthreads();
 }
 
 template <int PT>
@@ -107,7 +145,8 @@
   FrameState *fs = kp.state + b;
   const float *frame = kp.depth + (size_t)b * kp.g.D;
   const uint32_t n = kp.g.P;
-  const float U0 = bracket_hi_float(fs->brU[0]), L1 = bracket_lo_float(fs->brL[1]);
+  const ScanBounds bd = scan_bounds(fs);
+  const float U0 = bd.U0, L1 = bd.L1;
   const uint32_t q0 = (uint32_t)__cvta_generic_to_shared(&sm.pq[0][tid]);
   uint32_t qaddr = q0;
   const uint32_t tile_base = tile * (uint32_t)kTilePx;
@@ -133,7 +172,10 @@
     }
   }
   const uint32_t nq = (qaddr - q0) / (uint32_t)(kScanThreads * 4);
-  scan_flush(&sm.pq[0][0], nq, U0, L1, fs, kp, b, sm.flush);
+  uint32_t tails = 0;
+  scan_flush(&sm.pq[0][0], nq, bd, fs, kp, b, sm.flush, tails);
+  __syncthreads();
+  scan_tails_commit(tails, fs, sm.flush);
 }
 
 __device__ __forceinline__ void finalise_fast(FrameState *fs, uint32_t n) {
@@ -161,18 +203,32 @@
   vfs->status = D2PC_FRAME_READY;
 }
 
+template <int U, typename F4, typename F1>
+__device__ __forceinline__ void walk_queue(const float *q, uint32_t m, F4 f4, F1 f1) {
+  const uint32_t stride = blockDim.x, m4 = m >> 2;
+  const float4 *q4 = reinterpret_cast<const float4 *>(q);
+  uint32_t i = threadIdx.x;
+  for (; i + (uint32_t)(U - 1) * stride < m4; i += (uint32_t)U * stride) {
+    float4 v[U];
+#pragma unroll
+    for (int k = 0; k < U; ++k) v[k] = __ldcg(q4 + i + (uint32_t)k * stride);
+#pragma unroll
+    for (int k = 0; k < U; ++k) f4(v[k], i + (uint32_t)k * stride);
+  }
+  for (; i < m4; i += stride) f4(__ldcg(q4 + i), i);
+  const uint32_t r = (m4 << 2) + threadIdx.x;
+  if (r < m) f1(__ldcg(q + r), r);
+}
 template <int U, typename F>
 __device__ __forceinline__ void for_each_queued(const float *q, uint32_t nq, F f) {
-  const uint32_t stride = blockDim.x;
-  uint32_t i = threadIdx.x;
-  for (; i + (uint32_t)(U - 1) * stride < nq; i += (uint32_t)U * stride) {
-    float v[U];
-#pragma unroll
-    for (int k = 0; k < U; ++k) v[k] = __ldcg(q + i + (uint32_t)k * stride);
-#pragma unroll
-    for (int k = 0; k < U; ++k) f(v[k]);
-  }
-  for (; i < nq; i += stride) f(__ldcg(q + i));
+  walk_queue<U>(q, nq, [&](float4 v, uint32_t) { f(v.x); f(v.y); f(v.z); f(v.w); }, [&](float v, uint32_t) { f(v); });
+}
+
+constexpr int kQueueLoads = 4;
+
+__device__ __forceinline__ uint32_t bracket_below(volatile FrameState *vfs, int br, uint32_t n, uint32_t nqueue,
+                                                  uint32_t queued_below) {
+  return br == 0 ? vfs->below0 + queued_below : n - nqueue - vfs->above1;
 }
 
 constexpr int kSelectSmemWords = (int)kFastBins + 2 * (int)kFastListCap;
@@ -208,7 +264,7 @@
   __syncthreads();
   {
     uint32_t c_eqL = 0, c_in = 0, c_eqU = 0, c_below = 0, c_nf = 0;
-    for_each_queued<8>(q, nq, [&](float v) {
+    for_each_queued<kQueueLoads>(q, nq, [&](float v) {
       if (!(fabsf(v) < __int_as_float(0x7F800000))) c_nf += 1u + ((v != v) ? 0x10000u : 0u);
       else if (v < Lf) c_below++;
       else if (v == Lf) c_eqL++;
@@ -231,7 +287,7 @@
   }
   __syncthreads();
   const uint32_t eqL = ss.c[0], nin = ss.c[1], eqU = ss.c[2], n_nf = ss.c[4];
-  const uint32_t below = br == 0 ? ss.c[3] : n - nqueue;
+  const uint32_t below = bracket_below(vfs, br, n, nqueue, ss.c[3]);
   bool fail = (n_nf != 0u) || (nqueue > qcap) || (fs->sample_ok == 0u) || (kp.force_fallback != 0);
   RankPair rp = percentile_ranks(n, br ? D2PC_Q98 : D2PC_Q02);
   bool want[2] = {false, false};
@@ -259,7 +315,7 @@
     } else if (!slow) {
       const bool shared_bin = want[0] && want[1] && bin[0] == bin[1];
       const bool own[2] = {want[0], want[1] && !shared_bin};
-      for_each_queued<8>(q, nq, [&](float v) {
+      for_each_queued<kQueueLoads>(q, nq, [&](float v) {
         if (v > Lf && v < Uf) {
           const uint32_t k = float_to_key(v);
           const uint32_t bk = (k - lo0) >> shift;
@@ -293,7 +349,7 @@
       uint32_t rk[2], ok_[2];
       for (int t = 0; t < 2; ++t) rk[t] = want[t] ? need[t] : need[1 - t];
       const bool ok = block_hist_select<2, 11>([&](auto f) {
-        for_each_queued<8>(q, nq, [&](float v) {
+        for_each_queued<kQueueLoads>(q, nq, [&](float v) {
           if (v > Lf && v < Uf) f(float_to_key(v));
         });
       }, lo0, hi0, rk, ok_, s_hist, ss.res);
@@ -307,7 +363,6 @@
     fs->sel_key[2 * br + 0] = key[0];
     fs->sel_key[2 * br + 1] = key[1];
     fs->eqL[br] = eqL; fs->inside[br] = nin; fs->eqU[br] = eqU;
-    fs->below[br] = below;
     if (n_nf) { atomicAdd(&fs->n_nonfinite, n_nf); atomicAdd(&fs->n_nan, ss.c[5]); }
     if (fail) atomicOr(&fs->sel_fail, 1u);
     __threadfence();
@@ -398,14 +453,14 @@
   c.hi0 = c.U < 0xFFFFFFFFu ? c.U + 1u : c.U;
   c.span = c.hi0 - c.lo0;
   c.shift = fast_shift(c.span);
-  const uint32_t chunk = (c.nq + K - 1u) / K;
+  const uint32_t chunk = ((c.nq + K - 1u) / K + 3u) & ~3u;
   c.s_lo = min(c.nq, k * chunk);
   c.m = min(c.nq, c.s_lo + chunk) - c.s_lo;
   c.cached = chunk <= slice_cap;
   return c;
 }
 
-template <bool LOCAL_HIST = false>
+template <bool LOCAL_HIST = false, int NLD = kQueueLoads>
 __device__ __forceinline__ int select_phase_a(const KParams &kp, int b, int br, uint32_t k, uint32_t K, float *s_slice,
                                               uint32_t slice_cap, SelPartSmall &ss) {
   const int tid = threadIdx.x, nthr = blockDim.x;
@@ -435,22 +490,13 @@
         if (d <= span) atomicAdd(&hist[d >> shift], 1u);
       } else if (v == Uf) c_eqU++;
     };
-    uint32_t i = tid;
-    for (; i + 7u * nthr < m; i += 8u * nthr) {
-      float v[8];
-#pragma unroll
-      for (int u = 0; u < 8; ++u) v[u] = __ldcg(q + s_lo + i + (uint32_t)u * nthr);
-#pragma unroll
-      for (int u = 0; u < 8; ++u) {
-        if (cached) s_slice[i + (uint32_t)u * nthr] = v[u];
-        visit(v[u]);
-      }
-    }
-    for (; i < m; i += nthr) {
-      const float v = __ldcg(q + s_lo + i);
+    walk_queue<NLD>(q + s_lo, m, [&](float4 v, uint32_t i4) {
+      if (cached) reinterpret_cast<float4 *>(s_slice)[i4] = v;
+      visit(v.x); visit(v.y); visit(v.z); visit(v.w);
+    }, [&](float v, uint32_t i) {
       if (cached) s_slice[i] = v;
       visit(v);
-    }
+    });
     c_eqL = warp_sum(c_eqL); c_in = warp_sum(c_in); c_eqU = warp_sum(c_eqU); c_below = warp_sum(c_below);
     const uint32_t w_nf = warp_sum(c_nf & 0xFFFFu), w_nan = warp_sum(c_nf >> 16);
     if ((tid & 31) == 0) {
@@ -484,7 +530,7 @@
   if (last_a) {
     volatile uint32_t *cn = sh->counts[br];
     const uint32_t eqL = cn[1], nin = cn[2], eqU = cn[3], n_nf = cn[4];
-    const uint32_t below = br == 0 ? cn[0] : n - nqueue;
+    const uint32_t below = bracket_below(fs, br, n, nqueue, cn[0]);
     bool fail = (n_nf != 0u) || (nqueue > qcap) || (fs->sample_ok == 0u) || (kp.force_fallback != 0);
     const RankPair rp = percentile_ranks(n, br ? D2PC_Q98 : D2PC_Q02);
     bool want[2] = {false, false};
@@ -531,6 +577,7 @@
   return 0;
 }
 
+template <int NLD = kQueueLoads>
 __device__ __forceinline__ void select_phase_c(const KParams &kp, int b, int br, uint32_t k, uint32_t K,
                                                float *s_slice, uint32_t slice_cap, bool slice_is_cached, SelPartSmall &ss) {
   const int tid = threadIdx.x, nthr = blockDim.x;
@@ -561,17 +608,10 @@
           }
       }
     };
-    uint32_t i = tid;
-    if (!cached) {
-      for (; i + 7u * nthr < m; i += 8u * nthr) {
-        float v[8];
-#pragma unroll
-        for (int u = 0; u < 8; ++u) v[u] = __ldcg(q + s_lo + i + (uint32_t)u * nthr);
-#pragma unroll
-        for (int u = 0; u < 8; ++u) collect(v[u]);
-      }
-    }
-    for (; i < m; i += nthr) collect(cached ? s_slice[i] : __ldcg(q + s_lo + i));
+    if (cached)
+      for (uint32_t i = tid; i < m; i += nthr) collect(s_slice[i]);
+    else
+      for_each_queued<NLD>(q + s_lo, m, collect);
   }
   __syncthreads();
   if (tid == 0) {
@@ -611,7 +651,7 @@
       uint32_t rk[2], ok_[2];
       for (int t = 0; t < 2; ++t) rk[t] = want[t] ? vsh->need[br][t] : vsh->need[br][1 - t];
       const bool ok = block_hist_select<2, 11>([&](auto f) {
-        for_each_queued<8>(q, nq, [&](float v) {
+        for_each_queued<NLD>(q, nq, [&](float v) {
           if (v > Lf && v < Uf) f(float_to_key(v));
         });
       }, lo0, hi0, rk, ok_, reinterpret_cast<uint32_t *>(s_slice), ss.res);
@@ -623,10 +663,10 @@
   }
 }
 
-template <typename Spin>
+template <int NLD = kQueueLoads, typename Spin>
 __device__ __forceinline__ bool select_part(const KParams &kp, int b, int br, uint32_t k, uint32_t K, float *s_slice,
                                             uint32_t slice_cap, SelPartSmall &ss, Spin spin) {
-  const int st = select_phase_a<false>(kp, b, br, k, K, s_slice, slice_cap, ss);
+  const int st = select_phase_a<false, NLD>(kp, b, br, k, K, s_slice, slice_cap, ss);
   if (st == 2) return true;
   SelShared *sh = kp.sel + b;
   if (st == 0) {
@@ -636,7 +676,7 @@
     if (*reinterpret_cast<volatile uint32_t *>(&sh->bin_ready[br]) == 2u) return true;
   }
   __syncthreads();
-  select_phase_c(kp, b, br, k, K, s_slice, slice_cap, true, ss);
+  select_phase_c<NLD>(kp, b, br, k, K, s_slice, slice_cap, true, ss);
   return true;
 }
 
diff --git a/profiles/micro/read_ceiling.cu b/profiles/micro/read_ceiling.cu
--- /dev/null
+++ b/profiles/micro/read_ceiling.cu
@@ -0,0 +1,35 @@
+#include <cstdint>
+#include <cuda_runtime.h>
+
+__device__ __forceinline__ float4 ld_first(const float4 *p, uint64_t pol) {
+  float4 r;
+  asm volatile("ld.global.nc.L1::no_allocate.L2::cache_hint.v4.f32 {%0,%1,%2,%3}, [%4], %5;"
+               : "=f"(r.x), "=f"(r.y), "=f"(r.z), "=f"(r.w) : "l"(p), "l"(pol));
+  return r;
+}
+
+template <int U>
+__global__ void __launch_bounds__(256) read_kernel(const float4 *src, float *sink) {
+  uint64_t pol;
+  asm("createpolicy.fractional.L2::evict_first.b64 %0, 1.0;" : "=l"(pol));
+  const float4 *p = src + (size_t)blockIdx.x * (256 * U) + threadIdx.x;
+  float4 r[U];
+#pragma unroll
+  for (int j = 0; j < U; ++j) r[j] = ld_first(p + j * 256, pol);
+  float s = 0.0f;
+#pragma unroll
+  for (int j = 0; j < U; ++j) s += r[j].x + r[j].y + r[j].z + r[j].w;
+  if (s == -1.0f) *sink = s;
+}
+
+extern "C" int read_stream_launch(const void *src, size_t n4, float *sink, int u, void *stream) {
+  cudaStream_t st = (cudaStream_t)stream;
+  const float4 *s = (const float4 *)src;
+  switch (u) {
+    case 4: read_kernel<4><<<(unsigned)(n4 / (256 * 4)), 256, 0, st>>>(s, sink); break;
+    case 8: read_kernel<8><<<(unsigned)(n4 / (256 * 8)), 256, 0, st>>>(s, sink); break;
+    case 16: read_kernel<16><<<(unsigned)(n4 / (256 * 16)), 256, 0, st>>>(s, sink); break;
+    default: return (int)cudaErrorInvalidValue;
+  }
+  return (int)cudaGetLastError();
+}
diff --git a/profiles/read_ceiling.py b/profiles/read_ceiling.py
--- /dev/null
+++ b/profiles/read_ceiling.py
@@ -0,0 +1,72 @@
+import ctypes
+import json
+import os
+import subprocess
+import sys
+import tempfile
+
+import torch
+
+HERE = os.path.dirname(os.path.abspath(__file__))
+
+
+def build(tmp):
+    nvcc = os.environ.get("NVCC") or "/usr/local/cuda/bin/nvcc"
+    so = os.path.join(tmp, "libreadceil.so")
+    subprocess.run([nvcc, "-gencode", "arch=compute_100a,code=sm_100a", "-O3", "-Xcompiler", "-fPIC", "-shared",
+                    "-o", so, os.path.join(HERE, "micro", "read_ceiling.cu")], check=True)
+    return ctypes.CDLL(so)
+
+
+def card():
+    try:
+        q = subprocess.run(["nvidia-smi", "--query-gpu=name,power.limit", "--format=csv,noheader"],
+                           capture_output=True, text=True, check=True).stdout.strip().splitlines()[0]
+        name, power = [x.strip() for x in q.split(",")]
+    except (OSError, subprocess.CalledProcessError, IndexError, ValueError):
+        name, power = torch.cuda.get_device_name(0), "unknown"
+    return name, power
+
+
+def timed(fn, iters):
+    for _ in range(3):
+        fn()
+    a, b = torch.cuda.Event(enable_timing=True), torch.cuda.Event(enable_timing=True)
+    torch.cuda.synchronize()
+    a.record()
+    for _ in range(iters):
+        fn()
+    b.record()
+    torch.cuda.synchronize()
+    return a.elapsed_time(b) / iters
+
+
+def main(gib=2.0, iters=50):
+    dev = torch.device("cuda", 0)
+    n4 = int(gib * (1 << 30)) // 16 // 4096 * 4096
+    buf = torch.rand(n4 * 4, device=dev)
+    sink = torch.zeros(1, device=dev)
+    nbytes = n4 * 16
+    out = {"bytes": nbytes, "iters": iters}
+    with tempfile.TemporaryDirectory() as tmp:
+        lib = build(tmp)
+        lib.read_stream_launch.argtypes = [ctypes.c_void_p, ctypes.c_size_t, ctypes.c_void_p, ctypes.c_int,
+                                           ctypes.c_void_p]
+        st = torch.cuda.current_stream(dev).cuda_stream
+        for u in (4, 8, 16):
+            def run(u=u):
+                rc = lib.read_stream_launch(buf.data_ptr(), n4, sink.data_ptr(), u, st)
+                if rc:
+                    raise RuntimeError("read_stream_launch: cudaError %d" % rc)
+            ms = timed(run, iters)
+            out["stream_u%d_gbs" % u] = round(nbytes / ms / 1e6, 1)
+    ms = timed(lambda: torch.sum(buf), iters)
+    out["torch_sum_gbs"] = round(nbytes / ms / 1e6, 1)
+    out["ceiling_gbs"] = max(v for k, v in out.items() if k.endswith("_gbs"))
+    out["card"], out["power_limit"] = card()
+    print(json.dumps(out))
+
+
+if __name__ == "__main__":
+    a = sys.argv[1:]
+    main(float(a[0]) if a else 2.0, int(a[1]) if len(a) > 1 else 50)
diff --git a/profiles/stats_only.py b/profiles/stats_only.py
--- a/profiles/stats_only.py
+++ b/profiles/stats_only.py
@@ -1,3 +1,4 @@
+import json
 import os
 import sys
 
@@ -7,12 +8,21 @@
 import image_to_pointcloud_b200 as m
 
 
-def main(batch=128, iters=20, H=1080, W=1920, h=None, w=None):
+def make_depth(batch, h, w, dev, scene):
+    g = torch.Generator(device=dev)
+    g.manual_seed(7)
+    if not scene:
+        return torch.rand((batch, h, w), generator=g, device=dev) * 20
+    vv, uu = torch.meshgrid(torch.arange(h, device=dev), torch.arange(w, device=dev), indexing="ij")
+    r = torch.hypot(uu - w / 2.0, vv - h / 2.0) / w
+    base = 20.0 / (1.0 + r)
+    return (base + torch.randn((batch, h, w), generator=g, device=dev) * 0.01).float().contiguous()
+
+
+def main(batch=128, iters=20, H=1080, W=1920, h=None, w=None, kernels=False, scene=False):
     dev = torch.device("cuda", 0)
     h, w = h or H, w or W
-    g = torch.Generator(device=dev)
-    g.manual_seed(7)
-    depth = torch.rand((batch, h, w), generator=g, device=dev) * 20
+    depth = make_depth(batch, h, w, dev, scene)
     eng = m.FrameEngine(H, W, h, w, batch=batch, device=dev)
     cfg = eng.make_config(density="high")
     s = torch.cuda.current_stream(dev)
@@ -27,9 +37,31 @@
     torch.cuda.synchronize()
     eng.enqueue_status(cfg, s)
     torch.cuda.synchronize()
-    print("stats ms per %d frames: %.4f  (any fallback: %d)" % (batch, a.elapsed_time(b) / iters, int(eng._any_host[0])))
+    n_fb = int(sum(1 for p in eng.frame_params(cfg) if p["status"] != 1))
+    out = {"batch": batch, "img": [H, W], "depth": [h, w], "scene": scene,
+           "stats_ms": round(a.elapsed_time(b) / iters, 4), "fallback_frames": n_fb}
+    if kernels:
+        from torch.profiler import ProfilerActivity, profile
+        with profile(activities=[ProfilerActivity.CUDA]) as prof:
+            for _ in range(iters):
+                eng.enqueue_stats(cfg, depth, s)
+            torch.cuda.synchronize()
+        per = {}
+        for e in prof.events():
+            if e.device_type == torch.autograd.DeviceType.CUDA:
+                name = e.name.split("(")[0].replace("void ", "").replace("d2pc::", "")
+                per[name] = per.get(name, 0.0) + e.time_range.elapsed_us() / iters
+        out["kernels_us"] = {k: round(v, 2) for k, v in sorted(per.items(), key=lambda kv: -kv[1])}
+    return out
 
 
 if __name__ == "__main__":
-    a = [int(x) for x in sys.argv[1:]]
-    main(*a)
+    flags = {a for a in sys.argv[1:] if a.startswith("--")}
+    a = [int(x) for x in sys.argv[1:] if not x.startswith("--")]
+    r = main(*a, kernels="--kernels" in flags, scene="--scene" in flags)
+    if "--json" in flags:
+        print(json.dumps(r))
+    else:
+        print("stats ms per %d frames: %.4f  (fallback frames: %d)" % (r["batch"], r["stats_ms"], r["fallback_frames"]))
+        for k, v in r.get("kernels_us", {}).items():
+            print("  %-60s %9.2f us" % (k, v))
```

New measurement: 172,400, median of 6. About the same (-0.7%).
